# hongfz16/AvatarCLIP

Hardware: AMD Instinct MI355X
Metric: rays_per_sec_512x512_64spp_clip_guided_train_iter (higher is better)
Workload: dtype f16 (forward) / bf16 (gradient sweeps) MFMA operands, fp32 accumulate

## Files before the change

avatarclip_amd/csrc/avc_bwd_body.h:

```cpp
#pragma once
#include "avc_mlp.h"
constexpr int BWD_G = 4;
constexpr int BWD_WPB = 8;

template <typename P> __device__ __forceinline__ P launder(P p) {
  asm volatile("" : "+s"(p));
  return p;
}
template <typename V>
__device__ __forceinline__ V zero_frag() {
  V z;
#pragma unroll
  for (int j = 0; j < 8; ++j) z[j] = (typename MF<V>::S)0.f;
  return z;
}
__device__ __forceinline__ float second_term(float gbar_h, float g_a, float s) {
  const float r = s > 1e-30f ? __builtin_amdgcn_rcpf(s) : 0.f;
  return gbar_h * g_a * (AVC_BETA * (1.f - s) * r);
}
struct PF3 { h8 h0, h1; b8 b0, b1; h8 g0, g1; };

struct BwdArgs {
  PointSrc ps;
  long npts;
  const b8* Wb0;
  const float* T0;
  const float* d_sdf;
  const float* d_normal;
  const float* d_rgb;
  const float* rgb_fwd;
  const char* fpanels;
  char* gpanels;
  const unsigned short* masks;
  float* colsum;
};

#define AVC_CS_DUMMY 64
template <class N> struct ColSum {
  static constexpr int SLOT_FLOATS = PanelLayout<N>::CS_FLOATS + AVC_CS_DUMMY;
  static constexpr int LDS_BYTES = BWD_WPB * SLOT_FLOATS * 4;
};
typedef AVC_LDS float* cs_slot_t;
__device__ __forceinline__ float quad_xor1(float x) {
  return __builtin_bit_cast(float, __builtin_amdgcn_update_dpp(0, __builtin_bit_cast(int, x), 0xB1, 0xf, 0xf, true));
}
__device__ __forceinline__ float quad_xor2(float x) {
  return __builtin_bit_cast(float, __builtin_amdgcn_update_dpp(0, __builtin_bit_cast(int, x), 0x4E, 0xf, 0xf, true));
}
template <int NV>
__device__ __forceinline__ float transpose_sum(const float (&v)[NV], int lane) {
  static_assert(NV == 8 || NV == 16, "8 or 16 values per lane");
  float w[NV / 2];
  const bool b0 = lane & 1, b1 = lane & 2, b2 = lane & 4, b3 = lane & 8;
#pragma unroll
  for (int k = 0; k < NV / 2; ++k) w[k] = (b0 ? v[2 * k + 1] : v[2 * k]) + quad_xor1(b0 ? v[2 * k] : v[2 * k + 1]);
  float x[NV / 4];
#pragma unroll
  for (int k = 0; k < NV / 4; ++k) x[k] = (b1 ? w[2 * k + 1] : w[2 * k]) + quad_xor2(b1 ? w[2 * k] : w[2 * k + 1]);
  float y[NV / 8];
#pragma unroll
  for (int k = 0; k < NV / 8; ++k) y[k] = (b2 ? x[2 * k + 1] : x[2 * k]) + __shfl_xor(b2 ? x[2 * k] : x[2 * k + 1], 4);
  float z;
  if constexpr (NV == 16) z = (b3 ? y[1] : y[0]) + __shfl_xor(b3 ? y[0] : y[1], 8);
  else z = y[0] + __shfl_xor(y[0], 8);
  return z + __shfl_xor(z, 16);
}
template <class N, int NV>
__device__ __forceinline__ void col_sums(cs_slot_t slot, int lane, int base, const float (&v)[NV]) {
  const float total = transpose_sum<NV>(v, lane);
  const bool writer = (lane & 31) < NV;
  cs_slot_t dst = writer ? slot + base + (lane & (NV - 1)) : slot + PanelLayout<N>::CS_FLOATS + (lane & 63);
  *dst = *dst + total;
}
template <class N>
__device__ __forceinline__ cs_slot_t cs_init(char* lds_base, int wv, int lane) {
  cs_slot_t slot = (cs_slot_t)lds_base + wv * ColSum<N>::SLOT_FLOATS;
  for (int k = lane; k < ColSum<N>::SLOT_FLOATS; k += 64) slot[k] = 0.f;
  return slot;
}
template <class N>
__device__ __forceinline__ void cs_flush(cs_slot_t slot, float* out, long row, int lane) {
  asm volatile("s_waitcnt lgkmcnt(0)" ::: "memory");
  for (int k = lane; k < PanelLayout<N>::CS_FLOATS; k += 64) out[row * PanelLayout<N>::CS_FLOATS + k] = slot[k];
}

template <class N> struct BlkIn { b8 dof; unsigned m1[N::HT], m2[N::HT]; float dn[3], dsdf; };
template <class N>
__device__ __forceinline__ void load_blk_in(const BwdArgs& a, long blk, long nblk, int lane, BlkIn<N>& bi) {
  typedef PanelLayout<N> L;
  const int h = lane >> 5, p = lane & 31;
  long i = blk * 32 + p;
  const float vmask = i < a.npts ? 1.f : 0.f;
  if (i >= a.npts) i = a.npts - 1;
  bi.dof = zero_frag<b8>();
#pragma unroll
  for (int r = 0; r < 4; ++r) {
    const int ch = h ? 4 + r : r;
    const float c = (ch < 6) ? a.rgb_fwd[6 * i + (ch < 6 ? ch : 0)] : 0.f;
    const float dr = (ch < 6) ? a.d_rgb[6 * i + (ch < 6 ? ch : 0)] * vmask : 0.f;
    bi.dof[r] = (__bf16)(dr * c * (1.f - c));
  }
  const AVC_GLOBAL unsigned short* mk = as_global(a.masks) + (blk < nblk ? blk : nblk) * (long)L::MASK_U16 + lane;
#pragma unroll
  for (int t = 0; t < N::HT; ++t) {
    bi.m1[t] = mk[t * 64];
    bi.m2[t] = (N::NCMID == 1) ? mk[(N::HT + t) * 64] : 0u;
  }
#pragma unroll
  for (int c = 0; c < 3; ++c) bi.dn[c] = a.d_normal[3 * i + c] * vmask;
  bi.dsdf = a.d_sdf[i] * vmask;
}

struct NoRing {
  static constexpr bool on = false;
  template <class N> __device__ __forceinline__ void handoff(int, const b8 (&)[N::HK], long, int, int) const {}
};

template <class N, bool PIPE = false, class R>
__device__ __forceinline__ void bwd_sweeps(StageT<BWD_G>& sg, const BwdArgs& a, lds_tab_t Tl, long blk0, long nblk, int lane0,
                                           int wv, R& ring, cs_slot_t cs, BlkIn<N>* bip = nullptr, long blk0_next = 0) {
  typedef PanelLayout<N> L;
  constexpr AvcOffsets o = Off<N>::value;
  const PointSrc& ps = a.ps;
  const long npts = a.npts;
  const b8* Wb = launder(a.Wb0);
  lds_tab_t T = Tl;
  asm volatile("" : "+s"(T));
  int lane = lane0;
  asm volatile("" : "+v"(lane));
  const int h = lane >> 5, p = lane & 31;
  sg.lane = lane;
  const long blk = blk0 + wv;
  const long bsel = blk < nblk ? blk : nblk;
  const PanelPtr ftiles = panel_ptr(const_cast<char*>(a.fpanels) + bsel * (long)L::P_TILES * 2048, lane);
  const PanelPtr tiles = panel_ptr(a.gpanels + bsel * (long)L::G_TILES * 2048, lane);
  long i = blk * 32 + p;
  const bool valid = i < npts;
  if (!valid) i = npts - 1;
  const float vmask = valid ? 1.f : 0.f;
  float x[3];
  fetch_point(ps, i, x);
  float nbar[3];
  float dsdf_in;
  {
    BlkIn<N> bi_local;
    if constexpr (!PIPE) load_blk_in<N>(a, blk, nblk, lane, bi_local);
    BlkIn<N>& bi = PIPE ? *bip : bi_local;
    b8 dof[1];
    dof[0] = bi.dof;
    tile_store<false>(tiles, L::G_DO, dof[0], zero_frag<b8>());
    unsigned m1[N::HT], m2[N::HT];
#pragma unroll
    for (int t = 0; t < N::HT; ++t) { m1[t] = bi.m1[t]; m2[t] = bi.m2[t]; }
    const float dn_in[3] = {bi.dn[0], bi.dn[1], bi.dn[2]};
    dsdf_in = bi.dsdf;
#define AVC_RELU_BWD(OUT, MSK, PT)                                                                         \
  AVC_EPI(const unsigned bits = MSK[t];                                                                      \
          _Pragma("unroll") for (int j = 0; j < 8; ++j) {                                                    \
            OUT[2 * t][j] = (__bf16)(((bits >> relu_mask_bit(j)) & 1u) ? acc[j] : 0.f);                      \
            OUT[2 * t + 1][j] = (__bf16)(((bits >> relu_mask_bit(8 + j)) & 1u) ? acc[8 + j] : 0.f); }        \
          pin2(OUT[2 * t], OUT[2 * t + 1]);                                                                  \
          tile_store<false>(tiles, (PT) + t, OUT[2 * t], OUT[2 * t + 1]);)
    b8 dl[N::HK];
    b8 d1[N::HK];
    if constexpr (N::NCMID == 1) {
      layer_s1<b8, 1, N::HT>(sg, Wb, o.v[OFF_CHT], nxt<N, OFF_CM0T>(sg, Wb, o), dof, AVC_RELU_BWD(dl, m2, L::G_D2));
      layer_s1<b8, N::HK, N::HT>(sg, Wb, o.v[OFF_CM0T], nxt<N, OFF_C0T>(sg, Wb, o), dl, AVC_RELU_BWD(d1, m1, L::G_D1));
    } else {
      layer_s1<b8, 1, N::HT>(sg, Wb, o.v[OFF_CHT], nxt<N, OFF_C0T>(sg, Wb, o), dof, AVC_RELU_BWD(d1, m1, L::G_D1));
    }
    float dn_acc[3] = {0.f, 0.f, 0.f};
    layer_s1<b8, N::HK, N::HT + 1>(sg, Wb, o.v[OFF_C0T], nxt<N, OFF_W0G>(sg, Wb, o), d1, AVC_EPI(
      if (t < N::HT) {
        b8 f0, f1;
        _Pragma("unroll") for (int j = 0; j < 8; ++j) { f0[j] = (__bf16)acc[j]; f1[j] = (__bf16)acc[8 + j]; }
        pin2(f0, f1);
        tile_store<true>(tiles, L::G_DFEAT + (t < N::HT ? t : 0), f0, f1);
      } else {
        dn_acc[0] = acc[3]; dn_acc[1] = acc[0]; dn_acc[2] = acc[1];
      }
    ));
    {
      const float a3 = dn_acc[0], a0 = dn_acc[1], a1 = dn_acc[2];
      const float o3 = __shfl_xor(a3, 32), o0 = __shfl_xor(a0, 32), o1 = __shfl_xor(a1, 32);
      nbar[0] = valid ? dn_in[0] + (h ? o3 : a3) : 0.f;
      nbar[1] = valid ? dn_in[1] + (h ? a0 : o0) : 0.f;
      nbar[2] = valid ? dn_in[2] + (h ? a1 : o1) : 0.f;
    }
  }
  const float dsdf = dsdf_in;
  const float dsdfS = dsdf * AVC_S;
  {
    b8 fs = zero_frag<b8>();
    if (h == 0) {
      fs[0] = (__bf16)dsdf;
      fs[1] = (__bf16)(dsdf - (float)fs[0]);
    }
    tile_store<false>(tiles, L::G_SDF, fs, zero_frag<b8>());
  }
  b8 gbs[N::SK];
  b8 dfeat[N::HK];
  auto load_dfeat = [&]() __attribute__((always_inline)) {
#pragma unroll
    for (int t = 0; t < N::HT; ++t) {
      const FragPair<b8> d = tile_load<true, b8>(tiles, L::G_DFEAT + t);
      dfeat[2 * t] = d.a0;
      dfeat[2 * t + 1] = d.a1;
    }
  };
  {
    b8 gb0[3];
    {
      PE pe4;
      pe_compute(x, h, pe4);
      float g0[24];
#pragma unroll
      for (int q = 0; q < 24; ++q) {
        g0[q] = pe4.d[q] * nbar[q % 3];
        gb0[q >> 3][q & 7] = (__bf16)g0[q];
      }
#pragma unroll
      for (int s = 0; s < 3; ++s) {
        float v[8];
#pragma unroll
        for (int j = 0; j < 8; ++j) v[j] = g0[8 * s + j];
        col_sums<N, 8>(cs, lane, N::ST * 32 + (s * 2 + h) * 8, v);
      }
    }
    tile_store<false>(tiles, L::G_GB0, gb0[0], gb0[1]);
    tile_store<false>(tiles, L::G_GB0 + 1, gb0[2], zero_frag<b8>());
#define AVC_E_LOADH(PH) tile_load<false, h8>(ftiles, (PH) + t)
#define AVC_SECOND(OUT, PH, PT)                                                                              \
  AVC_PRE(return AVC_E_LOADH(PH);),                                                                          \
  AVC_EPID(FragPair<h8>, _Pragma("unroll") for (int j = 0; j < 8; ++j) {                                     \
            OUT[2 * t][j] = (__bf16)(acc[j] * sig_from_h((float)d.a0[j]));                                   \
            OUT[2 * t + 1][j] = (__bf16)(acc[8 + j] * sig_from_h((float)d.a1[j])); }                         \
          pin2(OUT[2 * t], OUT[2 * t + 1]);                                                                  \
          tile_store<true>(tiles, (PT) + t, OUT[2 * t], OUT[2 * t + 1]);)
#define AVC_SECOND_S(OUT, PH)                                                                                \
  AVC_PRE(return AVC_E_LOADH(PH);),                                                                          \
  AVC_EPID(FragPair<h8>, float v[16];                                                                        \
          _Pragma("unroll") for (int j = 0; j < 8; ++j) {                                                    \
            v[j] = acc[j] * sig_from_h((float)d.a0[j]);                                                      \
            v[8 + j] = acc[8 + j] * sig_from_h((float)d.a1[j]);                                              \
            OUT[2 * t][j] = (__bf16)v[j];                                                                    \
            OUT[2 * t + 1][j] = (__bf16)v[8 + j]; }                                                          \
          pin2(OUT[2 * t], OUT[2 * t + 1]);                                                                  \
          col_sums<N, 16>(cs, lane, (t * 2 + h) * 16, v);)
    b8 gb1[N::HK];
    layer_sq1<b8, 3, N::HT>(sg, Wb, o.v[OFF_W0G], nxt<N, OFF_WM0>(sg, Wb, o), gb0, AVC_SECOND(gb1, L::P_H1, L::G_GBH1));
    b8 gbm[N::HK];
    if constexpr (N::NMID == 2) {
      layer_sq1<b8, N::HK, N::HT>(sg, Wb, o.v[OFF_WM0], nxt<N, OFF_WM1>(sg, Wb, o), gb1, AVC_SECOND(gbm, L::P_HM, L::G_GBHM));
      b8 gbm1[N::HK];
      layer_sq1<b8, N::HK, N::HT>(sg, Wb, o.v[OFF_WM1], nxt<N, OFF_WS>(sg, Wb, o), gbm,
                                  AVC_SECOND(gbm1, L::P_HM + N::HT, L::G_GBHM + N::HT));
      layer_sq1<b8, N::HK, N::ST>(sg, Wb, o.v[OFF_WS], nxt<N, OFF_WLT>(sg, Wb, o), gbm1, AVC_SECOND_S(gbs, L::P_HS));
    } else {
      layer_sq1<b8, N::HK, N::HT>(sg, Wb, o.v[OFF_WM0], nxt<N, OFF_WS>(sg, Wb, o), gb1, AVC_SECOND(gbm, L::P_HM, L::G_GBHM));
      layer_sq1<b8, N::HK, N::ST>(sg, Wb, o.v[OFF_WS], nxt<N, OFF_WLT>(sg, Wb, o), gbm, AVC_SECOND_S(gbs, L::P_HS));
    }
  }
  {
    b8 as_[N::SK];
    load_dfeat();
#define AVC_F_LOADB(PB) tile_load<true, b8>(tiles, (PB) + t)
#define AVC_LOAD3(PH, PB, PG)                                                                               \
  AVC_PRE(PF3 d; { const FragPair<h8> a_ = tile_load<true, h8>(ftiles, (PH) + t); d.h0 = a_.a0; d.h1 = a_.a1; } \
          { const FragPair<b8> a_ = AVC_F_LOADB(PB); d.b0 = a_.a0; d.b1 = a_.a1; } \
          { const FragPair<h8> a_ = tile_load<true, h8>(ftiles, (PG) + t); d.g0 = a_.a0; d.g1 = a_.a1; } return d;)
#define AVC_LOAD3_S(PH, PG)                                                                                 \
  AVC_PRE(PF3 d; { const FragPair<h8> a_ = tile_load<true, h8>(ftiles, (PH) + t); d.h0 = a_.a0; d.h1 = a_.a1; } \
          d.b0 = gbs[2 * t]; d.b1 = gbs[2 * t + 1];                                                          \
          { const FragPair<h8> a_ = tile_load<true, h8>(ftiles, (PG) + t); d.g0 = a_.a0; d.g1 = a_.a1; } return d;)
    layer_sq1<b8, N::HK, N::ST>(sg, Wb, o.v[OFF_WLT], nxt<N, OFF_WST>(sg, Wb, o), dfeat,
      AVC_LOAD3_S(L::P_HS, L::P_GAS), AVC_EPID(PF3,
      float wa[16];
      load16(T + o.v[OFF_WL0_ACC], t, h, wa);
      _Pragma("unroll") for (int j = 0; j < 8; ++j) {
        const float s0 = sig_from_h((float)d.h0[j]), s1 = sig_from_h((float)d.h1[j]);
        as_[2 * t][j] = (__bf16)(second_term((float)d.b0[j], (float)d.g0[j], s0) + (acc[j] + wa[j] * dsdfS) * s0);
        as_[2 * t + 1][j] = (__bf16)(second_term((float)d.b1[j], (float)d.g1[j], s1) + (acc[8 + j] + wa[8 + j] * dsdfS) * s1);
      }
      pin2(as_[2 * t], as_[2 * t + 1]);
      tile_store<false>(tiles, L::G_ABS + t, as_[2 * t], as_[2 * t + 1]);
    ));
#define AVC_REVERSE(OUT, PH, PB, PG, PT, RINGED)                                                            \
  AVC_LOAD3(PH, PB, PG),                                                                                     \
  AVC_EPID(PF3, _Pragma("unroll") for (int j = 0; j < 8; ++j) {                                              \
            const float s0 = sig_from_h((float)d.h0[j]), s1 = sig_from_h((float)d.h1[j]);                    \
            OUT[2 * t][j] = (__bf16)(second_term((float)d.b0[j], (float)d.g0[j], s0) + acc[j] * s0);         \
            OUT[2 * t + 1][j] = (__bf16)(second_term((float)d.b1[j], (float)d.g1[j], s1) + acc[8 + j] * s1); } \
          pin2(OUT[2 * t], OUT[2 * t + 1]);                                                                  \
          if constexpr (!(RINGED)) tile_store<false>(tiles, (PT) + t, OUT[2 * t], OUT[2 * t + 1]);)
    b8 am[N::HK];
    b8 am0[N::HK];
    const Next first = nxt<N, OFF_CHT>(sg, a.Wb0, o);
#define AVC_F_LASTHOOK AVC_HOOK(if constexpr (PIPE) load_blk_in<N>(a, blk0_next + wv, nblk, lane, *bip);)
    if constexpr (N::NMID == 2) {
      layer_sq1<b8, N::SK, N::HT>(sg, Wb, o.v[OFF_WST], nxt<N, OFF_WM1T>(sg, Wb, o), as_,
                                 AVC_REVERSE(am, L::P_HM + N::HT, L::G_GBHM + N::HT, L::P_GAM + N::HT, L::G_ABM + N::HT, R::on));
      if constexpr (R::on) ring.template handoff<N>(1, am, blk0, lane, wv);
      layer_sq1<b8, N::HK, N::HT>(sg, Wb, o.v[OFF_WM1T], nxt<N, OFF_WM0T>(sg, Wb, o), am,
                                 AVC_REVERSE(am0, L::P_HM, L::G_GBHM, L::P_GAM, L::G_ABM, R::on));
      if constexpr (R::on) ring.template handoff<N>(0, am0, blk0, lane, wv);
      layer_sq1<b8, N::HK, N::HT>(sg, Wb, o.v[OFF_WM0T], first, am0, AVC_REVERSE(am, L::P_H1, L::G_GBH1, L::P_GA1, L::G_AB1, false), AVC_F_LASTHOOK);
    } else {
      layer_sq1<b8, N::SK, N::HT>(sg, Wb, o.v[OFF_WST], nxt<N, OFF_WM0T>(sg, Wb, o), as_,
                                 AVC_REVERSE(am, L::P_HM, L::G_GBHM, L::P_GAM, L::G_ABM, R::on));
      if constexpr (R::on) ring.template handoff<N>(0, am, blk0, lane, wv);
      layer_sq1<b8, N::HK, N::HT>(sg, Wb, o.v[OFF_WM0T], first, am, AVC_REVERSE(am0, L::P_H1, L::G_GBH1, L::P_GA1, L::G_AB1, false), AVC_F_LASTHOOK);
    }
  }
#undef AVC_RELU_BWD
#undef AVC_SECOND
#undef AVC_LOAD3
#undef AVC_LOAD3_S
#undef AVC_F_LOADB
#undef AVC_E_LOADH
#undef AVC_SECOND_S
#undef AVC_F_LASTHOOK
#undef AVC_REVERSE
}
```

avatarclip_amd/csrc/avc_mlp_bwd.hip:

```cpp
#include "avc_bwd_body.h"
#include "../../include/avc.h"

template <class N>
__global__ __launch_bounds__(64 * BWD_WPB) void mlp_bwd_kernel(BwdArgs a) {
  extern __shared__ __attribute__((aligned(16))) char lds[];
  typedef StageT<BWD_G> ST;
  constexpr AvcOffsets o = Off<N>::value;
  static_assert(BWD_WPB >= 4 && BWD_WPB % 4 == 0, "stage_issue's turns need a multiple of 4 wavefronts per workgroup");
  const int lane0 = threadIdx.x & 63;
  const int wv = threadIdx.x >> 6;
  const long nblk = (a.npts + 31) >> 5;
  ST sg = stage_init<BWD_G>(lds);
  stage_issue(sg, nxt<N, OFF_CHT>(sg, a.Wb0, o), 0);
  const lds_tab_t Tl = tab_to_lds(lds + ST::LDS_BYTES, a.T0, o.v[OFF_TAB_END]);
  const cs_slot_t cs = cs_init<N>(lds + ST::LDS_BYTES + AVC_TAB_LDS_BYTES, wv, lane0);
  __syncthreads();
  NoRing ring;
  BlkIn<N> bi;
  load_blk_in<N>(a, (long)blockIdx.x * BWD_WPB + wv, nblk, lane0, bi);
  for (long blk0 = (long)blockIdx.x * BWD_WPB; blk0 < nblk; blk0 += (long)gridDim.x * BWD_WPB)
    bwd_sweeps<N, true>(sg, a, Tl, blk0, nblk, lane0, wv, ring, cs, &bi, blk0 + (long)gridDim.x * BWD_WPB);
  cs_flush<N>(cs, a.colsum, (long)blockIdx.x * BWD_WPB + wv, lane0);
}

extern "C" int avc_bwd_colsum_floats(int net) { return net == AVC_NET_FULL ? PanelLayout<NetFull>::CS_FLOATS : PanelLayout<NetSmall>::CS_FLOATS; }
extern "C" long avc_bwd_colsum_rows(long npts, long max_waves) {
  const long nblk = (npts + 31) / 32;
  long ngroups = (nblk + BWD_WPB - 1) / BWD_WPB, maxg = max_waves / BWD_WPB;
  if (maxg < 1) maxg = 1;
  long grid = ngroups < maxg ? ngroups : maxg;
  if (grid < 1) grid = 1;
  return grid * BWD_WPB;
}

extern "C" int avc_render_points_bwd(int net, const float* pts, const float* rays_o, const float* rays_d, const float* z,
                                     int S, int ldz, float sample_dist, long npts, const void* wbf16, const float* tab,
                                     const int* offs, const float* d_sdf, const float* d_normal, const float* d_rgb,
                                     const float* rgb_fwd, const void* fpanels, void* gpanels, const void* masks, float* colsum,
                                     long max_waves, void* stream) {
  if (npts <= 0) return 0;
  if (!fpanels || !gpanels || !masks || !rgb_fwd || !colsum) { avc_set_error("avc_render_points_bwd: fpanels / gpanels / masks / rgb_fwd / colsum == NULL"); return 1; }
  if (!(net == AVC_NET_FULL ? offsets_match<NetFull>(offs) : offsets_match<NetSmall>(offs))) {
    avc_set_error("packed-blob offsets differ from the compiled-in table (regenerate csrc/avc_offsets_gen.h)");
    return 1;
  }
  PointSrc ps{pts, rays_o, rays_d, z, S, ldz, pts ? 0 : 1, sample_dist};
  const long nblk = (npts + 31) / 32;
  long ngroups = (nblk + BWD_WPB - 1) / BWD_WPB;
  long maxg = max_waves / BWD_WPB;
  if (maxg < 1) maxg = 1;
  int grid = (int)(ngroups < maxg ? ngroups : maxg);
  if (grid < 1) grid = 1;
  hipStream_t s = (hipStream_t)stream;
  const int lds_bytes = StageT<BWD_G>::LDS_BYTES + AVC_TAB_LDS_BYTES + ColSum<NetFull>::LDS_BYTES;
  if (offs[OFF_TAB_END] * 4 > AVC_TAB_LDS_BYTES) { avc_set_error("fp32 table does not fit its LDS window"); return 1; }
  static unsigned long long attr_seen = 0;
  if (avc_first_use_on_device(attr_seen)) {
    (void)hipFuncSetAttribute((const void*)mlp_bwd_kernel<NetFull>, hipFuncAttributeMaxDynamicSharedMemorySize, lds_bytes);
    (void)hipFuncSetAttribute((const void*)mlp_bwd_kernel<NetSmall>, hipFuncAttributeMaxDynamicSharedMemorySize, lds_bytes);
  }
  const BwdArgs args{ps, npts, (const b8*)wbf16, tab, d_sdf, d_normal, d_rgb, rgb_fwd, (const char*)fpanels, (char*)gpanels,
                     (const unsigned short*)masks, colsum};
  if (net == AVC_NET_FULL)
    hipLaunchKernelGGL((mlp_bwd_kernel<NetFull>), dim3(grid), dim3(64 * BWD_WPB), lds_bytes, s, args);
  else if (net == AVC_NET_SMALL)
    hipLaunchKernelGGL((mlp_bwd_kernel<NetSmall>), dim3(grid), dim3(64 * BWD_WPB), lds_bytes, s, args);
  else { avc_set_error("unknown net id"); return 1; }
  return avc_check_launch("avc_render_points_bwd");
}
```

avatarclip_amd/csrc/avc_wgrad.hip:

```cpp
#include "avc_common.h"
#include "../../include/avc.h"

#include "avc_wgrad_body.h"

template <int NI, int NK>
__device__ __forceinline__ void weight_grad_body(char* lds, const WgRegions& rg, int pa, int ta_n, int pb,
                                                 int tb_n, int type_a, int type_b, long nblk, float* __restrict__ partial,
                                                 float* __restrict__ bias_partial, int out_elems, int bias_elems, int WA) {
  const int lane = threadIdx.x & 63;
  const int wv = __builtin_amdgcn_readfirstlane((int)(threadIdx.x >> 6));
  const int WB = 8 / WA;
  const int wa = wv % WA, wb = wv / WA;
  const int split = blockIdx.x, nsplit = gridDim.x;
  const long b0 = nblk * split / nsplit, b1 = nblk * (split + 1) / nsplit;
  const int ntile = ta_n + tb_n;
  const int nchunk = ntile * 2;
  const int my_chunks = (nchunk - wv + 7) >> 3;
  constexpr int slot_bytes = WG_BUF_BYTES, depth = WG_DEPTH;
  const int src_lo = ((lane >> 2) & 3) * 32 + 4 * (lane >> 4) + (lane & 3);
  const char* const base_a = (type_a ? rg.base[1] : rg.base[0]) + (long)pa * 2048;
  const char* const base_b = (type_b ? rg.base[1] : rg.base[0]) + (long)pb * 2048;
  const long stride_a = type_a ? rg.stride[1] : rg.stride[0], stride_b = type_b ? rg.stride[1] : rg.stride[0];
  auto issue = [&](long blk, int slot) {
    for (int c = wv; c < nchunk; c += 8) {
      const int tix = c >> 1;
      const char* tb_ = tix < ta_n ? base_a + blk * stride_a + (long)tix * 2048 : base_b + blk * stride_b + (long)(tix - ta_n) * 2048;
      const char* g = tb_ + (src_lo + (c & 1) * 16) * 16;
      __builtin_amdgcn_global_load_lds((const __attribute__((address_space(1))) void*)g,
                                       (__attribute__((address_space(3))) void*)(lds + slot * slot_bytes + c * 1024), 16, 0, WG_DMA_AUX);
    }
  };
  const int lane_off = (((lane >> 5) * 2) * 16 + (((lane >> 4) & 1) * 2 + (lane & 1)) * 4 + ((lane & 15) >> 2)) * 16 + 8 * ((lane & 3) >> 1);
  facc acc[NI * NK];
#pragma unroll
  for (int q = 0; q < NI * NK; ++q)
#pragma unroll
    for (int r = 0; r < 16; ++r) acc[q][r] = 0.f;
  float bsum[NI];
#pragma unroll
  for (int i = 0; i < NI; ++i) bsum[i] = 0.f;
  for (int d = 0; d < depth - 1; ++d)
    if (b0 + d < b1) issue(b0 + d, d);
  int slot = 0;
  for (long blk = b0; blk < b1; ++blk) {
    long younger = b1 - 1 - blk;
    if (younger > depth - 2) younger = depth - 2;
    wait_vmcnt((int)younger * my_chunks);
    asm volatile("s_waitcnt lgkmcnt(0)" ::: "memory");
    __builtin_amdgcn_s_barrier();
    __builtin_amdgcn_sched_barrier(0);
    if (blk + depth - 1 < b1) { int ns = slot + depth - 1; if (ns >= depth) ns -= depth; issue(blk + depth - 1, ns); }
    lds_char* buf = (lds_char*)(lds + slot * slot_bytes) + lane_off;
    b8 a[NI][2];
#pragma unroll
    for (int i = 0; i < NI; ++i) {
      const int ta = wa + WA * i;
      if (ta < ta_n) {
        a[i][0] = tr_frag(buf + ta * 2048, 0);
        a[i][1] = tr_frag(buf + ta * 2048, 1);
      }
    }
    b8 bv[NK][2];
#pragma unroll
    for (int k = 0; k < NK; ++k) {
      const int tb = wb + WB * k;
      if (tb < tb_n) {
        bv[k][0] = tr_frag(buf + (ta_n + tb) * 2048, 0);
        bv[k][1] = tr_frag(buf + (ta_n + tb) * 2048, 1);
      }
    }
    if (type_a == 0) {
#pragma unroll
      for (int i = 0; i < NI; ++i) { a[i][0] = f16_to_bf16(a[i][0]); a[i][1] = f16_to_bf16(a[i][1]); }
    }
    if (type_b == 0) {
#pragma unroll
      for (int k = 0; k < NK; ++k) { bv[k][0] = f16_to_bf16(bv[k][0]); bv[k][1] = f16_to_bf16(bv[k][1]); }
    }
#pragma unroll
    for (int i = 0; i < NI; ++i) {
      if (wa + WA * i < ta_n) {
        if (bias_partial && wb == i) {
#pragma unroll
          for (int j = 0; j < 8; ++j) bsum[i] += (float)a[i][0][j] + (float)a[i][1][j];
        }
#pragma unroll
        for (int k = 0; k < NK; ++k) {
          if (wb + WB * k < tb_n) {
            acc[i * NK + k] = MF<b8>::mma(a[i][0], bv[k][0], acc[i * NK + k]);
            acc[i * NK + k] = MF<b8>::mma(a[i][1], bv[k][1], acc[i * NK + k]);
          }
        }
      }
    }
    if (++slot == depth) slot = 0;
  }
  float* dst = partial + (long)split * out_elems;
#pragma unroll
  for (int i = 0; i < NI; ++i) {
    const int ta = wa + WA * i;
    if (ta >= ta_n) continue;
#pragma unroll
    for (int k = 0; k < NK; ++k) {
      const int tb = wb + WB * k;
      if (tb >= tb_n) continue;
      f4* d4 = reinterpret_cast<f4*>(dst + ((long)(ta * tb_n + tb) * 64 + lane) * 16);
#pragma unroll
      for (int q = 0; q < 4; ++q) {
        f4 v;
        v[0] = acc[i * NK + k][4 * q]; v[1] = acc[i * NK + k][4 * q + 1]; v[2] = acc[i * NK + k][4 * q + 2]; v[3] = acc[i * NK + k][4 * q + 3];
        d4[q] = v;
      }
    }
    if (bias_partial && wb == i) {
      const float s = xhalf_sum(bsum[i]);
      if (lane < 32) bias_partial[(long)split * bias_elems + ta * 32 + lane] = s;
    }
  }
}

__device__ __forceinline__ void weight_grad_body_9x9(char* lds, const WgRegions& rg, int pa, int pb, int type_a,
                                                     int type_b, long nblk, float* __restrict__ partial,
                                                     float* __restrict__ bias_partial, int out_elems, int bias_elems) {
  constexpr int TA = 9, TB = 9, NT = TA + TB;
  const int lane = threadIdx.x & 63;
  const int wv = __builtin_amdgcn_readfirstlane((int)(threadIdx.x >> 6));
  const int wa = wv & 3, wb = wv >> 2;
  const int split = blockIdx.x, nsplit = gridDim.x;
  const long b0 = nblk * split / nsplit, b1 = nblk * (split + 1) / nsplit;
  constexpr int nchunk = NT * 2;
  const int my_chunks = (nchunk - wv + 7) >> 3;
  const int src_lo = ((lane >> 2) & 3) * 32 + 4 * (lane >> 4) + (lane & 3);
  const char* const base_a = (type_a ? rg.base[1] : rg.base[0]) + (long)pa * 2048;
  const char* const base_b = (type_b ? rg.base[1] : rg.base[0]) + (long)pb * 2048;
  const long stride_a = type_a ? rg.stride[1] : rg.stride[0], stride_b = type_b ? rg.stride[1] : rg.stride[0];
  auto issue = [&](long blk, int slot) {
    for (int c = wv; c < nchunk; c += 8) {
      const int tix = c >> 1;
      const char* tb_ = tix < TA ? base_a + blk * stride_a + (long)tix * 2048 : base_b + blk * stride_b + (long)(tix - TA) * 2048;
      const char* g = tb_ + (src_lo + (c & 1) * 16) * 16;
      __builtin_amdgcn_global_load_lds((const __attribute__((address_space(1))) void*)g,
                                       (__attribute__((address_space(3))) void*)(lds + slot * WG_BUF_BYTES + c * 1024), 16, 0, WG_DMA_AUX);
    }
  };
  const int lane_off = (((lane >> 5) * 2) * 16 + (((lane >> 4) & 1) * 2 + (lane & 1)) * 4 + ((lane & 15) >> 2)) * 16 + 8 * ((lane & 3) >> 1);
  facc acc[10], ex[2];
#pragma unroll
  for (int q = 0; q < 10; ++q)
#pragma unroll
    for (int r = 0; r < 16; ++r) acc[q][r] = 0.f;
#pragma unroll
  for (int q = 0; q < 2; ++q)
#pragma unroll
    for (int r = 0; r < 16; ++r) ex[q][r] = 0.f;
  float bsum[2] = {0.f, 0.f}, xsum = 0.f;
  const bool has_x = wb == 1 || wa == 0;
  const int xk = wb == 1 ? wa : 4;
  for (int d = 0; d < WG_DEPTH - 1; ++d)
    if (b0 + d < b1) issue(b0 + d, d);
  int slot = 0;
  for (long blk = b0; blk < b1; ++blk) {
    long younger = b1 - 1 - blk;
    if (younger > WG_DEPTH - 2) younger = WG_DEPTH - 2;
    wait_vmcnt((int)younger * my_chunks);
    asm volatile("s_waitcnt lgkmcnt(0)" ::: "memory");
    __builtin_amdgcn_s_barrier();
    __builtin_amdgcn_sched_barrier(0);
    if (blk + WG_DEPTH - 1 < b1) issue(blk + WG_DEPTH - 1, (slot + WG_DEPTH - 1) % WG_DEPTH);
    lds_char* buf = (lds_char*)(lds + slot * WG_BUF_BYTES) + lane_off;
    auto load_b = [&](int tb, b8& f0, b8& f1) {
      f0 = tr_frag(buf + (TA + tb) * 2048, 0);
      f1 = tr_frag(buf + (TA + tb) * 2048, 1);
    };
    b8 a[2][2], sa[2], c0, c1, n0, n1;
    load_b(wb, c0, c1);
    n0 = c0; n1 = c1;
#pragma unroll
    for (int i = 0; i < 2; ++i) {
      a[i][0] = tr_frag(buf + (wa + 4 * i) * 2048, 0);
      a[i][1] = tr_frag(buf + (wa + 4 * i) * 2048, 1);
    }
    if (has_x) { sa[0] = tr_frag(buf + 8 * 2048, 0); sa[1] = tr_frag(buf + 8 * 2048, 1); }
    if (type_a == 0) {
#pragma unroll
      for (int i = 0; i < 2; ++i) { a[i][0] = f16_to_bf16(a[i][0]); a[i][1] = f16_to_bf16(a[i][1]); }
      if (has_x) { sa[0] = f16_to_bf16(sa[0]); sa[1] = f16_to_bf16(sa[1]); }
    }
    if (bias_partial) {
#pragma unroll
      for (int i = 0; i < 2; ++i)
        if (wb == i) {
#pragma unroll
          for (int j = 0; j < 8; ++j) bsum[i] += (float)a[i][0][j] + (float)a[i][1][j];
        }
    }
    if (bias_partial && wv == 4) {
#pragma unroll
      for (int j = 0; j < 8; ++j) xsum += (float)sa[0][j] + (float)sa[1][j];
    }
#pragma unroll
    for (int k = 0; k < 6; ++k) {
      const int tb_next = (k + 1 < 5) ? wb + 2 * (k + 1) : 2 * wa;
      const bool next_ok = (k + 1 < 5) ? (tb_next < TB) : (k + 1 == 5 && wb == 1);
      if (next_ok) load_b(tb_next, n0, n1);
      asm volatile("" : "+v"(n0), "+v"(n1));
      const bool cur_ok = (k < 5) ? (wb + 2 * k < TB) : (wb == 1);
      if (cur_ok) {
        if (type_b == 0) { c0 = f16_to_bf16(c0); c1 = f16_to_bf16(c1); }
        if (k < 5) {
          acc[k] = MF<b8>::mma(a[0][0], c0, acc[k]);
          acc[k] = MF<b8>::mma(a[0][1], c1, acc[k]);
          acc[5 + k] = MF<b8>::mma(a[1][0], c0, acc[5 + k]);
          acc[5 + k] = MF<b8>::mma(a[1][1], c1, acc[5 + k]);
          if (has_x && k == xk) {
            ex[0] = MF<b8>::mma(sa[0], c0, ex[0]);
            ex[0] = MF<b8>::mma(sa[1], c1, ex[0]);
          }
        } else {
          ex[1] = MF<b8>::mma(sa[0], c0, ex[1]);
          ex[1] = MF<b8>::mma(sa[1], c1, ex[1]);
        }
      }
      c0 = n0; c1 = n1;
    }
    slot = (slot + 1) % WG_DEPTH;
  }
  float* dst = partial + (long)split * out_elems;
  auto store_tile = [&](int ta, int tb, const facc& v16) {
    f4* d4 = reinterpret_cast<f4*>(dst + ((long)(ta * TB + tb) * 64 + lane) * 16);
#pragma unroll
    for (int q = 0; q < 4; ++q) {
      f4 v;
      v[0] = v16[4 * q]; v[1] = v16[4 * q + 1]; v[2] = v16[4 * q + 2]; v[3] = v16[4 * q + 3];
      d4[q] = v;
    }
  };
#pragma unroll
  for (int k = 0; k < 5; ++k) {
    if (wb + 2 * k < TB) {
      store_tile(wa, wb + 2 * k, acc[k]);
      store_tile(wa + 4, wb + 2 * k, acc[5 + k]);
    }
  }
  if (has_x) store_tile(8, wb + 2 * xk, ex[0]);
  if (wb == 1) store_tile(8, 2 * wa, ex[1]);
  if (bias_partial) {
#pragma unroll
    for (int i = 0; i < 2; ++i) {
      if (wb == i) {
        const float sx = xhalf_sum(bsum[i]);
        if (lane < 32) bias_partial[(long)split * bias_elems + (wa + 4 * i) * 32 + lane] = sx;
      }
    }
    if (wv == 4) {
      const float sx = xhalf_sum(xsum);
      if (lane < 32) bias_partial[(long)split * bias_elems + 8 * 32 + lane] = sx;
    }
  }
}

#define WG_MAX_PAIRS 24
struct WgPairs { int v[WG_MAX_PAIRS][8]; };
__global__ __launch_bounds__(512) void weight_grad_all_kernel(WgRegions rg, WgPairs pp, long nblk,
                                                              float* __restrict__ partial, float* __restrict__ bias_partial,
                                                              int out_elems, int bias_elems) {
  extern __shared__ __attribute__((aligned(16))) char lds[];
  const int* d = pp.v[blockIdx.y];
  float* bp = d[5] >= 0 ? bias_partial + d[5] : nullptr;
#define WG_ARGS lds, rg, d[0], d[1], d[2], d[3], d[6], d[7], nblk, partial + d[4], bp, out_elems, bias_elems
  if (d[1] > 1 && d[3] > 2 && d[3] <= 8) {
    if (d[7] == 0) weight_grad_body<4, 2>(WG_ARGS, 2);
    else weight_grad_body<2, 4>(WG_ARGS, 4);
  } else if (d[1] == 9 && d[3] == 9) {
    weight_grad_body_9x9(lds, rg, d[0], d[2], d[6], d[7], nblk, partial + d[4], bp, out_elems, bias_elems);
  } else if (d[1] > 1 && d[3] > 8) {
    weight_grad_body<2, 5>(WG_ARGS, 4);
  } else if (d[1] > 1) {
    weight_grad_body<1, 2>(WG_ARGS, 8);
  } else {
    weight_grad_body<1, 2>(WG_ARGS, 1);
  }
#undef WG_ARGS
}

extern "C" int avc_weight_grad_all(const void* fpanels, int ftiles, const void* gpanels, int gtiles, int npairs, const int* pairs,
                                   long nblk, float* partial, float* bias_partial, int nsplit, int out_stride, int bias_stride,
                                   void* stream) {
  if (nblk <= 0 || npairs <= 0) return 0;
  if (!fpanels || !gpanels) { avc_set_error("avc_weight_grad_all: fpanels / gpanels == NULL"); return 1; }
  if (npairs > WG_MAX_PAIRS) { avc_set_error("avc_weight_grad_all: too many pairs"); return 1; }
  WgPairs pp;
  for (int i = 0; i < npairs; ++i) {
    for (int k = 0; k < 8; ++k) pp.v[i][k] = pairs[i * 8 + k];
    const bool merged = pp.v[i][1] == 9 && pp.v[i][3] == 9;
    if (!merged && (pp.v[i][1] < 1 || pp.v[i][1] > 8 || pp.v[i][3] < 1 || pp.v[i][3] > WG_TB_MAX)) {
      avc_set_error("avc_weight_grad_all: 1 <= ta <= 8, 1 <= tb <= 9 (or the 9 x 9 product)");
      return 1;
    }
  }
  if (nsplit < 1) nsplit = 1;
  const int lds_bytes = WG_DEPTH * WG_BUF_BYTES;
  static unsigned long long attr_seen = 0;
  if (avc_first_use_on_device(attr_seen)) {
    (void)hipFuncSetAttribute((const void*)weight_grad_all_kernel, hipFuncAttributeMaxDynamicSharedMemorySize, lds_bytes);
  }
  WgRegions rg;
  rg.base[0] = (const char*)fpanels; rg.stride[0] = (long)ftiles * 2048;
  rg.base[1] = (const char*)gpanels; rg.stride[1] = (long)gtiles * 2048;
  hipLaunchKernelGGL(weight_grad_all_kernel, dim3(nsplit, npairs), dim3(512), lds_bytes, (hipStream_t)stream, rg, pp, nblk, partial,
                     bias_partial, out_stride, bias_stride);
  return avc_check_launch("avc_weight_grad_all");
}

__global__ __launch_bounds__(256) void wgrad_reduce_kernel(const float* __restrict__ partial, const float* __restrict__ bpartial, int ns,
                                                           long stride, long bstride, int gout4, int gbias4, float* __restrict__ acc,
                                                           int accumulate) {
  const int j = blockIdx.x * 256 + threadIdx.x;
  if (j >= gout4 + gbias4) return;
  const f4* src = j < gout4 ? reinterpret_cast<const f4*>(partial) + j : reinterpret_cast<const f4*>(bpartial) + (j - gout4);
  const long st4 = (j < gout4 ? stride : bstride) >> 2;
  f4 a = {0.f, 0.f, 0.f, 0.f};
  int s = 0;
  for (; s + 8 <= ns; s += 8) {
    f4 v[8];
#pragma unroll
    for (int u = 0; u < 8; ++u) v[u] = __builtin_nontemporal_load(src + (long)(s + u) * st4);
#pragma unroll
    for (int u = 0; u < 8; ++u) a += v[u];
  }
  for (; s < ns; ++s) a += __builtin_nontemporal_load(src + (long)s * st4);
  f4* out = reinterpret_cast<f4*>(acc) + j;
  if (accumulate) a += *out;
  *out = a;
}
__global__ __launch_bounds__(256) void wgrad_unpack_kernel(const float* __restrict__ acc, const int* __restrict__ off, const int* __restrict__ src,
                                                           const float* __restrict__ scale, int nparam, float* __restrict__ grad) {
  const int t = blockIdx.x * 256 + threadIdx.x;
  if (t >= nparam) return;
  float g = 0.f;
  for (int k = off[t]; k < off[t + 1]; ++k) g += acc[src[k]] * scale[k];
  grad[t] = g;
}
extern "C" int avc_weight_grad_reduce(const float* partial, const float* bias_partial, int nsplit, int out_stride, int bias_stride,
                                      int gout_size, int gbias_size, float* acc, int accumulate, void* stream) {
  if ((gout_size & 3) || (gbias_size & 3) || (out_stride & 3) || (bias_stride & 3)) {
    avc_set_error("avc_weight_grad_reduce: sizes and strides must be multiples of 4 floats");
    return 1;
  }
  if (nsplit < 1 || !partial || !acc || (gbias_size && !bias_partial)) { avc_set_error("avc_weight_grad_reduce: bad arguments"); return 1; }
  const int n4 = (gout_size + gbias_size) / 4;
  hipLaunchKernelGGL(wgrad_reduce_kernel, dim3((n4 + 255) / 256), dim3(256), 0, (hipStream_t)stream, partial, bias_partial, nsplit,
                     (long)out_stride, (long)bias_stride, gout_size / 4, gbias_size / 4, acc, accumulate);
  return avc_check_launch("avc_weight_grad_reduce");
}
extern "C" int avc_weight_grad_unpack(const float* acc, const int* off, const int* src, const float* scale, int nparam, float* grad,
                                      void* stream) {
  if (nparam <= 0) return 0;
  if (!acc || !off || !src || !scale || !grad) { avc_set_error("avc_weight_grad_unpack: NULL buffer"); return 1; }
  hipLaunchKernelGGL(wgrad_unpack_kernel, dim3((nparam + 255) / 256), dim3(256), 0, (hipStream_t)stream, acc, off, src, scale, nparam, grad);
  return avc_check_launch("avc_weight_grad_unpack");
}
```

avatarclip_amd/engine.py:

```python
import ctypes
import os
import weakref

import numpy as np
import torch

from . import lib as L
from . import packing as PK


class _DevLayout:

    _cache = {}

    def __init__(self, lay: PK.Layout, device):
        t = lambda a, dt=None: torch.from_numpy(np.ascontiguousarray(a)).to(device)
        self.lay = lay
        self.idx16 = t(lay.idx16)
        self.scale16 = t(lay.scale16)
        self.idx32 = t(lay.idx32)
        self.scale32 = t(lay.scale32)
        self.un_src = t(lay.un_src)
        self.un_tgt = t(lay.un_tgt)
        self.un_scale = t(lay.un_scale)
        self.ub_src = t(lay.ub_src)
        self.ub_tgt = t(lay.ub_tgt)
        tgt = np.concatenate([lay.un_tgt, lay.ub_tgt]).astype(np.int64)
        src = np.concatenate([lay.un_src, np.asarray(lay.ub_src, np.int64) + lay.gout_size]).astype(np.int64)
        scl = np.concatenate([lay.un_scale, np.ones(len(lay.ub_tgt), np.float32)]).astype(np.float32)
        order = np.argsort(tgt, kind="stable")
        off = np.zeros(lay.nparam + 1, np.int64)
        np.cumsum(np.bincount(tgt, minlength=lay.nparam), out=off[1:])
        self.csr_off, self.csr_src, self.csr_scale = t(off.astype(np.int32)), t(src[order].astype(np.int32)), t(scl[order])
        self.cs_src, self.cs_tgt, self.cs_scale = t(lay.cs_src), t(lay.cs_tgt), t(lay.cs_scale)
        self._offsets_arr = (ctypes.c_int * PK.OFF_COUNT)(*[int(v) for v in lay.offsets])
        self.offsets = ctypes.cast(self._offsets_arr, ctypes.c_void_p)

    @classmethod
    def get(cls, spec, device):
        key = (spec.H, spec.NMID, spec.NCMID, str(device))
        if key not in cls._cache:
            cls._cache[key] = cls(PK.layout_for(spec), device)
        return cls._cache[key]


FUSED_PACK = os.environ.get("AVC_FUSED_PACK", "1") != "0"


class Packed:

    def __init__(self, dl: _DevLayout, flatP: torch.Tensor):
        self.dl = dl
        if flatP.is_cuda and FUSED_PACK:
            f = flatP.detach().float().contiguous()
            n16, n32 = dl.idx16.numel(), dl.idx32.numel()
            self.w_f16 = torch.empty(n16, dtype=torch.float16, device=f.device)
            self.w_bf16 = torch.empty(n16, dtype=torch.bfloat16, device=f.device)
            self.tab = torch.empty(n32, dtype=torch.float32, device=f.device)
            L.check(L.load().avc_pack_params(L.ptr(f), f.numel(), L.ptr(dl.idx16), L.ptr(dl.scale16), n16, L.ptr(dl.idx32), L.ptr(dl.scale32), n32,
                                             L.ptr(self.w_f16), L.ptr(self.w_bf16), L.ptr(self.tab), L.stream()), "avc_pack_params")
            return
        pz = torch.cat([flatP.detach().float(), flatP.new_zeros(1)])
        w = pz[dl.idx16] * dl.scale16
        self.w_f16 = w.to(torch.float16).contiguous()
        self.w_bf16 = w.to(torch.bfloat16).contiguous()
        self.tab = (pz[dl.idx32] * dl.scale32).contiguous()


def flatten_dense_torch(sdf_net, col_net, spec: PK.NetSpec) -> torch.Tensor:
    parts = []
    for W, b in sdf_net.dense():
        parts += [W.reshape(-1), b.reshape(-1)]
    if col_net is not None:
        for W, b in col_net.dense():
            parts += [W.reshape(-1), b.reshape(-1)]
    else:
        lay = PK.layout_for(spec)
        n_sdf = sum(int(np.prod(s)) for n, s in lay.shapes if n.startswith("sdf."))
        parts.append(parts[0].new_zeros(lay.nparam - n_sdf))
    return torch.cat(parts)


def _dense_layers(sdf_net, col_net, lay):
    out = []
    n_sdf = sdf_net.num_layers - 1
    for l in range(n_sdf):
        out.append((getattr(sdf_net, "lin%d" % l), lay.pbase["sdf.W%d" % l], lay.pbase["sdf.b%d" % l]))
    if col_net is not None:
        nh = col_net.num_layers - 2
        for l in range(nh):
            out.append((getattr(col_net, "lin%d" % l), lay.pbase["col.W%d" % l], lay.pbase["col.b%d" % l]))
        last = getattr(col_net, "lin%d" % nh)
        H = last.weight_v.shape[1] if hasattr(last, "weight_v") else last.weight.shape[1]
        out.append((last, lay.pbase["col.Wh"], lay.pbase["col.bh"]))
        if col_net.extra_color:
            out.append((col_net.extra_lin, lay.pbase["col.Wh"] + 3 * H, lay.pbase["col.bh"] + 3))
    return out


class DenseParamsFn(torch.autograd.Function):

    @staticmethod
    def forward(ctx, meta, *tensors):
        lay, offs = meta
        n = len(offs)
        dev = tensors[0].device
        flat = torch.zeros(lay.nparam, device=dev, dtype=torch.float32)
        vs, gs, bs = tensors[0::3], tensors[1::3], tensors[2::3]
        PA = ctypes.c_void_p * n
        arr = lambda ts: PA(*[(t.data_ptr() if t.numel() else None) for t in ts])
        ctx.rows = (ctypes.c_int * n)(*[v.shape[0] for v in vs])
        ctx.cols = (ctypes.c_int * n)(*[v.shape[1] for v in vs])
        ctx.w_off = (ctypes.c_long * n)(*[o[0] for o in offs])
        ctx.b_off = (ctypes.c_long * n)(*[o[1] for o in offs])
        ctx.n = n
        lib = L.load()
        assert all(t.is_contiguous() and t.dtype == torch.float32 for t in tensors)
        L.check(lib.avc_dense_params_fwd(n, arr(vs), arr(gs), arr(bs), ctx.rows, ctx.cols, ctx.w_off, ctx.b_off, L.ptr(flat), L.stream()),
                "avc_dense_params_fwd")
        ctx.save_for_backward(*tensors)
        return flat

    @staticmethod
    def backward(ctx, dflat):
        tensors = ctx.saved_tensors
        n = ctx.n
        vs, gs, bs = tensors[0::3], tensors[1::3], tensors[2::3]
        dflat = dflat.contiguous().float()
        outs = [torch.empty_like(t) for t in tensors]
        PA = ctypes.c_void_p * n
        arr = lambda ts: PA(*[(t.data_ptr() if t.numel() else None) for t in ts])
        L.check(L.load().avc_dense_params_bwd(n, arr(vs), arr(gs), arr(outs[0::3]), arr(outs[1::3]), arr(outs[2::3]), ctx.rows, ctx.cols,
                                              ctx.w_off, ctx.b_off, L.ptr(dflat), L.stream()), "avc_dense_params_bwd")
        return (None,) + tuple(o if t.numel() else None for o, t in zip(outs, tensors))


def flatten_dense(sdf_net, col_net, spec: PK.NetSpec) -> torch.Tensor:
    p0 = next(sdf_net.parameters())
    if p0.device.type != "cuda":
        return flatten_dense_torch(sdf_net, col_net, spec)
    lay = PK.layout_for(spec)
    tensors, offs = [], []
    empty = p0.new_zeros(0)
    for lin, w_off, b_off in _dense_layers(sdf_net, col_net, lay):
        if hasattr(lin, "weight_g"):
            tensors += [lin.weight_v, lin.weight_g, lin.bias if lin.bias is not None else empty]
        else:
            tensors += [lin.weight, empty, lin.bias if lin.bias is not None else empty]
        offs.append((int(w_off), int(b_off)))
    return DenseParamsFn.apply((lay, offs), *tensors)


def plan_panels(R, S, budget, blk_f, blk_g, slab_blocks, min_slab_blocks):
    nb = lambda rays: (rays * S + 31) // 32 + 1
    rays_of = lambda blocks: min(R, max(32, blocks * 32 // S // 32 * 32))
    blocks = slab_blocks
    slab = rays_of(blocks)
    while nb(R) * blk_f + nb(slab) * blk_g > budget and blocks > min_slab_blocks:
        blocks //= 2
        slab = rays_of(blocks)
    if nb(R) * blk_f + nb(slab) * blk_g <= budget:
        return R, slab
    if nb(slab) * (blk_f + blk_g) > budget:
        slab = max(32, (budget // (blk_f + blk_g) - 1) * 32 // S // 32 * 32)
    chunk = max(slab, ((budget - nb(slab) * blk_g) // blk_f - 1) * 32 // S // 32 * 32)
    return min(chunk, R), min(slab, R)


class Engine:
    _by_net = weakref.WeakKeyDictionary()
    PROFILE = False
    prof_events = []
    WG_BLOCKS_PER_SPLIT = int(os.environ.get("AVC_WG_BLOCKS_PER_SPLIT", "256"))
    WG_MAX_SPLITS = int(os.environ.get("AVC_WG_MAX_SPLITS", "256"))
    FUSED_WG_TAIL = os.environ.get("AVC_FUSED_WG_TAIL", "1") != "0"
    MAX_FWD_WAVES = 2048
    MAX_BWD_WAVES = 2048
    SDF_BIAS_FP32 = os.environ.get("AVC_SDF_BIAS_FP32", "1") != "0"
    RING = os.environ.get("AVC_BWD_RING", "0") != "0"
    RING_CPT = int(os.environ.get("AVC_RING_CPT", "2"))
    RING_SLOTS = int(os.environ.get("AVC_RING_SLOTS", "6"))
    RING_CHECK = os.environ.get("AVC_RING_CHECK", "0") != "0"
    PANEL_BYTES_BUDGET = int(os.environ.get("AVC_PANEL_GIB", "224")) << 30
    SLAB_BLOCKS = int(os.environ.get("AVC_SLAB_BLOCKS", str(512 * 1024)))
    MIN_SLAB_BLOCKS = 32 * 1024

    def __init__(self, spec: PK.NetSpec, device):
        if device.type != "cuda":
            raise RuntimeError("avatarclip_amd runs its hot path on an MI355X; got device %s (no CPU fallback)" % device)
        self.spec = spec
        self.device = device
        self.lib = L.load()
        self.dl = _DevLayout.get(spec, device)
        self.net = spec.net_id
        assert self.lib.avc_num_offsets() == PK.OFF_COUNT
        self.fwd_tiles = self.lib.avc_fwd_panel_tiles(self.net)
        self.grad_tiles = self.lib.avc_grad_panel_tiles(self.net)
        assert (self.fwd_tiles, self.grad_tiles) == (self.dl.lay.panel["FTILES"], self.dl.lay.panel["GTILES"]), \
            "panel layout mismatch between packing.py and csrc/avc_mlp.h"
        assert self.lib.avc_bwd_colsum_floats(self.net) == self.dl.lay.cs_size, "column-sum layout mismatch between packing.py and csrc/avc_mlp.h"
        self._colsum = None
        self.mask_u16 = self.lib.avc_mask_u16_per_block(self.net)
        self.fwd_scr_bytes = self.lib.avc_fwd_scratch_bytes_per_wave(self.net)
        self._fwd_scratch = None
        self._fpanels = None
        self._gpanels = None
        self._partials = None
        self._bpartials = None
        self._masks = None
        self._pairs_host = PK.region_local_pairs(self.dl.lay)
        self._sdf_bias0 = int(self.dl.lay.pbase["sdf.b%d" % (spec.NMID + 2)])
        self._packed_key = None
        self._packed = None
        self._panel_owner = None
        self._ring = None
        self.ring_stats = None

    @classmethod
    def for_networks(cls, sdf_net, col_net):
        eng = cls._by_net.get(sdf_net)
        if eng is None:
            col_conf = col_net.conf if col_net is not None else dict(
                d_hidden=sdf_net.conf["d_hidden"], n_layers=2 if sdf_net.conf["d_hidden"] == 256 else 1,
                mode="no_view_dir", multires_view=0)
            spec = PK.spec_from_conf(sdf_net.conf, col_conf)
            eng = cls(spec, next(sdf_net.parameters()).device)
            cls._by_net[sdf_net] = eng
        return eng

    class _Timed:
        def __init__(self, name, npts):
            self.name, self.npts = name, npts

        def __enter__(self):
            if Engine.PROFILE:
                self.e0 = torch.cuda.Event(enable_timing=True)
                self.e1 = torch.cuda.Event(enable_timing=True)
                self.e0.record()
            return self

        def __exit__(self, *a):
            if Engine.PROFILE:
                self.e1.record()
                Engine.prof_events.append((self.name, self.npts, self.e0, self.e1))
            return False

    def pack(self, flatP: torch.Tensor) -> Packed:
        last = getattr(self, "_last_pack", None)
        if last is not None and last[0]() is flatP and last[1] == flatP._version:
            return last[2]
        pk = Packed(self.dl, flatP)
        self._last_pack = (weakref.ref(flatP), flatP._version, pk)
        return pk

    def colsum_scratch(self):
        if getattr(self, "_colsum_scratch", None) is None:
            self._colsum_scratch = torch.zeros(self.lib.avc_colsum_scratch_bytes(), dtype=torch.uint8, device=self.device)
        return self._colsum_scratch

    def _grow(self, attr, nbytes, dtype=torch.uint8):
        buf = getattr(self, attr)
        esz = torch.empty(0, dtype=dtype).element_size()
        n = nbytes // esz
        if buf is None or buf.numel() < n:
            n = ((n * esz + (1 << 21) - 1) >> 21 << 21) // esz
            buf = None
            setattr(self, attr, None)
            torch.cuda.empty_cache()
            buf = torch.zeros(n, dtype=dtype, device=self.device)
            setattr(self, attr, buf)
        return buf

    def _bufs_f(self, nblk_chunk):
        return (self._grow("_fpanels", (nblk_chunk + 1) * self.fwd_tiles * 2048),
                self._grow("_masks", (nblk_chunk + 1) * self.mask_u16 * 2, torch.int16))

    def _bufs_g(self, nblk_slab):
        return self._grow("_gpanels", (nblk_slab + 1) * self.grad_tiles * 2048)

    def _ring_setup(self):
        if not L.has_ring():
            raise RuntimeError("AVC_BWD_RING=1 needs libavc_ring.so (python -m avatarclip_amd.build --ring; AVC_LIB_NAME=libavc_ring.so): the "
                               "role-specialised backward is an experiment that is not part of libavc.so (include/avc_ring.h)")
        key = (self.RING_CPT, self.RING_SLOTS)
        if self._ring is not None and self._ring["key"] == key:
            return self._ring
        lay, lib = self.dl.lay, self.lib
        ht = self.spec.H // 32
        ntypes = lib.avc_bwd_ring_types(self.net)
        assert ntypes == self.spec.NMID
        ring_rows, pb, offs = [], [], []
        for m in range(ntypes):
            row = [i for i, pr in enumerate(lay.pairs) if pr[0] == lay.panel["ABM"] + m * ht and pr[6] == 1]
            assert len(row) == 1
            pr = lay.pairs[row[0]]
            assert pr[1] == ht and pr[3] == ht and pr[7] == 0 and pr[5] >= 0, "ring products are HT x HT with an F-region B operand and a bias"
            ring_rows.append(row[0]); pb.append(int(pr[2])); offs.append((int(pr[4]), int(pr[5])))
        rest = np.ascontiguousarray(np.delete(self._pairs_host, ring_rows, axis=0))
        nrow = 8 * self.RING_CPT
        dev = self.device
        self._ring = dict(
            key=key, ntypes=ntypes, ht=ht, offs=offs, rest=rest,
            ctl=torch.zeros(lib.avc_bwd_ring_ctl_bytes() // 4, dtype=torch.int32, device=dev),
            payload=torch.empty(lib.avc_bwd_ring_payload_bytes(self.net, ntypes, self.RING_SLOTS), dtype=torch.uint8, device=dev),
            partial=torch.zeros(ntypes, nrow, ht * ht * 1024, dtype=torch.float32, device=dev),
            bias=torch.zeros(ntypes, nrow, ht * 32, dtype=torch.float32, device=dev),
            pb=(ctypes.c_int * ntypes)(*pb),
            err=torch.zeros((), dtype=torch.int32, device=dev),
            grid=torch.cuda.get_device_properties(dev).multi_processor_count)
        return self._ring

    def _held_bytes(self):
        return sum(b.numel() * b.element_size() for b in (self._fpanels, self._gpanels, self._masks) if b is not None)

    def plan(self, R, S):
        key = (R, S, self.PANEL_BYTES_BUDGET, self.SLAB_BLOCKS)
        if getattr(self, "_plan_key", None) == key:
            chunk, slab = self._plan_val
            if chunk < R or (self._fpanels is not None and self._fpanels.numel() >= ((R * S + 31) // 32 + 1) * self.fwd_tiles * 2048):
                return self._plan_val
        nb_all = (R * S + 31) // 32 + 1
        if (self._fpanels is not None and self._gpanels is not None and nb_all <= self.SLAB_BLOCKS
                and self._fpanels.numel() >= nb_all * self.fwd_tiles * 2048 and self._gpanels.numel() >= nb_all * self.grad_tiles * 2048
                and self._held_bytes() <= self.PANEL_BYTES_BUDGET):
            return R, R
        budget = max(min(self.PANEL_BYTES_BUDGET, (torch.cuda.mem_get_info(self.device)[0] + self._held_bytes()) * 8 // 10), 1 << 26)
        self._plan_key = key
        self._plan_val = plan_panels(R, S, budget, self.fwd_tiles * 2048 + self.mask_u16 * 2, self.grad_tiles * 2048,
                                     self.SLAB_BLOCKS, self.MIN_SLAB_BLOCKS)
        return self._plan_val

    def rays_per_chunk(self, R, S):
        return self.plan(R, S)[0]

    def sdf_rays(self, pk: Packed, rays_o, rays_d, z, sdf_out=None, slot=None, ld_out=0):
        R, S = z.shape
        if sdf_out is None:
            sdf_out = torch.empty(R, S, device=self.device, dtype=torch.float32)
        with Engine._Timed("avc_sdf_forward", R * S):
            L.check(self.lib.avc_sdf_forward(self.net, None, L.ptr(rays_o), L.ptr(rays_d), L.ptr(z), S, z.stride(0), R * S,
                                             L.ptr(pk.w_f16), L.ptr(pk.tab), self.dl.offsets, L.ptr(sdf_out),
                                             L.ptr(slot), ld_out, L.stream()), "avc_sdf_forward")
        return sdf_out

    def sdf_pts(self, pk: Packed, pts):
        pts = pts.contiguous().float()
        out = torch.empty(pts.shape[0], 1, device=self.device, dtype=torch.float32)
        L.check(self.lib.avc_sdf_forward(self.net, L.ptr(pts), None, None, None, 1, 1, pts.shape[0], L.ptr(pk.w_f16),
                                         L.ptr(pk.tab), self.dl.offsets, L.ptr(out), None, 0, L.stream()),
                "avc_sdf_forward")
        return out

    def upsample_step(self, rays_o, rays_d, z, sdf, m, inv_s):
        R, n = z.shape
        z_out = torch.empty(R, n + m, device=self.device, dtype=torch.float32)
        sdf_out = torch.empty(R, n + m, device=self.device, dtype=torch.float32)
        z_new = torch.empty(R, m, device=self.device, dtype=torch.float32)
        slot = torch.empty(R, m, device=self.device, dtype=torch.int32)
        lanes = 64 if os.environ.get("AVC_UPSAMPLE_GROUP", "1") == "0" else 0
        L.check(self.lib.avc_upsample_step_lanes(L.ptr(rays_o), L.ptr(rays_d), L.ptr(z), L.ptr(sdf), R, n, m, float(inv_s),
                                                 L.ptr(z_out), L.ptr(sdf_out), L.ptr(z_new), L.ptr(slot), lanes, L.stream()),
                "avc_upsample_step")
        return z_out, sdf_out, z_new, slot

    def points_fwd(self, pk: Packed, rays_o, rays_d, z, sample_dist):
        R, S = z.shape
        N = R * S
        sdf = torch.empty(R, S, device=self.device, dtype=torch.float32)
        nrm = torch.empty(R, S, 3, device=self.device, dtype=torch.float32)
        rgb = torch.empty(R, S, 6, device=self.device, dtype=torch.float32)
        if self._fwd_scratch is None:
            self._fwd_scratch = torch.empty(self.MAX_FWD_WAVES * self.fwd_scr_bytes, dtype=torch.uint8, device=self.device)
        with Engine._Timed("avc_render_points_fwd", N):
            L.check(self.lib.avc_render_points_fwd(self.net, None, L.ptr(rays_o), L.ptr(rays_d), L.ptr(z), S, z.stride(0),
                                                   float(sample_dist), N, L.ptr(pk.w_f16), L.ptr(pk.tab), self.dl.offsets,
                                                   L.ptr(sdf), L.ptr(nrm), L.ptr(rgb), self.MAX_FWD_WAVES, L.ptr(self._fwd_scratch),
                                                   L.stream()), "avc_render_points_fwd")
        return sdf, nrm, rgb

    def points_fwd_train(self, pk: Packed, rays_o, rays_d, z, sample_dist, r0=0, r1=None, out=None):
        R, S = z.shape
        r1 = R if r1 is None else r1
        if out is None:
            out = (torch.empty(R, S, device=self.device, dtype=torch.float32), torch.empty(R, S, 3, device=self.device, dtype=torch.float32),
                   torch.empty(R, S, 6, device=self.device, dtype=torch.float32))
        sdf, nrm, rgb = out
        npts = (r1 - r0) * S
        panels, masks = self._bufs_f((npts + 31) // 32)
        esz = 4
        with Engine._Timed("avc_render_points_fwd_train", npts):
            L.check(self.lib.avc_render_points_fwd_train(
                self.net, None, rays_o.data_ptr() + r0 * 3 * esz, rays_d.data_ptr() + r0 * 3 * esz,
                z.data_ptr() + r0 * z.stride(0) * esz, S, z.stride(0), float(sample_dist), npts, L.ptr(pk.w_f16), L.ptr(pk.tab),
                self.dl.offsets, sdf.data_ptr() + r0 * S * esz, nrm.data_ptr() + r0 * S * 3 * esz, rgb.data_ptr() + r0 * S * 6 * esz,
                self.MAX_FWD_WAVES, L.ptr(panels), L.ptr(masks), L.stream()), "avc_render_points_fwd_train")
        return out

    def composite_fwd(self, sdf, nrm, rgb, z, rays_o, rays_d, inv_s, sample_dist, cos_anneal, bg, bg_mode):
        R, S = z.shape
        dev, f32 = self.device, torch.float32
        color = torch.empty(R, 3, device=dev, dtype=f32)
        extra = torch.empty(R, 3, device=dev, dtype=f32)
        weights = torch.empty(R, S, device=dev, dtype=f32)
        cdf = torch.empty(R, S, device=dev, dtype=f32)
        mid_z = torch.empty(R, S, device=dev, dtype=f32)
        inside = torch.empty(R, S, device=dev, dtype=f32)
        eik = torch.empty(R, 2, device=dev, dtype=f32)
        wstat = torch.empty(2, R, device=dev, dtype=f32)
        nsum = torch.empty(R, 3, device=dev, dtype=f32)
        L.check(self.lib.avc_composite_fwd(L.ptr(sdf), L.ptr(nrm), L.ptr(rgb), L.ptr(z), L.ptr(rays_o), L.ptr(rays_d), R, S,
                                           L.ptr(inv_s), float(sample_dist), float(cos_anneal), L.ptr(bg), bg_mode,
                                           L.ptr(color), L.ptr(extra), L.ptr(weights), L.ptr(cdf), L.ptr(mid_z),
                                           L.ptr(inside), L.ptr(eik), L.ptr(wstat), L.ptr(nsum), L.stream()), "avc_composite_fwd")
        return color, extra, weights, cdf, mid_z, inside, eik, wstat, nsum

    def composite_bwd(self, sdf, nrm, rgb, z, rays_o, rays_d, inv_s, sample_dist, cos_anneal, bg, bg_mode, d_color,
                      d_extra, d_w, d_n_up, eik_scale, d_wsum=None, d_nsum=None):
        R, S = z.shape
        dev, f32 = self.device, torch.float32
        d_sdf = torch.empty(R, S, device=dev, dtype=f32)
        d_n = torch.empty(R, S, 3, device=dev, dtype=f32)
        d_rgb = torch.empty(R, S, 6, device=dev, dtype=f32)
        d_inv = torch.empty(R, device=dev, dtype=f32)
        L.check(self.lib.avc_composite_bwd(L.ptr(sdf), L.ptr(nrm), L.ptr(rgb), L.ptr(z), L.ptr(rays_o), L.ptr(rays_d), R, S,
                                           L.ptr(inv_s), float(sample_dist), float(cos_anneal), L.ptr(bg), bg_mode,
                                           L.ptr(d_color), L.ptr(d_extra), L.ptr(d_w), L.ptr(d_n_up), L.ptr(d_wsum), L.ptr(d_nsum),
                                           L.ptr(eik_scale), L.ptr(d_sdf), L.ptr(d_n), L.ptr(d_rgb), L.ptr(d_inv), L.stream()),
                "avc_composite_bwd")
        return d_sdf, d_n, d_rgb, d_inv

    def points_bwd(self, pk: Packed, rays_o, rays_d, z, sample_dist, d_sdf, d_n, d_rgb, rgb, panels_valid=False):
        lay = self.dl.lay
        R, S = z.shape
        rays_per_chunk, rays_per_slab = self.plan(R, S)
        if rays_per_chunk < R:
            panels_valid = False
        rg = self._ring_setup() if self.RING else None
        fused_tail = rg is None and self.FUSED_WG_TAIL and lay.gout_size % 4 == 0 and lay.gbias_size % 4 == 0
        if fused_tail:
            gacc = torch.empty(lay.gout_size + lay.gbias_size, device=self.device, dtype=torch.float32)
            nslab = 0
        else:
            gout = torch.zeros(lay.gout_size, device=self.device, dtype=torch.float32)
            gbias = torch.zeros(max(lay.gbias_size, 1), device=self.device, dtype=torch.float32)
        if self._partials is None:
            self._partials = torch.empty(256, lay.gout_size, device=self.device, dtype=torch.float32)
            self._bpartials = torch.empty(256, max(lay.gbias_size, 1), device=self.device, dtype=torch.float32)
        st = L.stream()
        esz = 4
        scratch_out = None
        if rg is not None:
            rg["err"].zero_()
        pairs_host = rg["rest"] if rg is not None else self._pairs_host
        cs_rows = int(self.lib.avc_bwd_colsum_rows(min(R, rays_per_slab) * S, self.MAX_BWD_WAVES)) if rg is None else 8 * rg["grid"]
        if self._colsum is None or self._colsum.shape[0] < cs_rows:
            self._colsum = torch.zeros(cs_rows, lay.cs_size, device=self.device, dtype=torch.float32)
        cs_total = None
        for c0 in range(0, R, rays_per_chunk):
            c1 = min(R, c0 + rays_per_chunk)
            if not panels_valid:
                if scratch_out is None:
                    scratch_out = (torch.empty(R, S, device=self.device), torch.empty(R, S, 3, device=self.device),
                                   torch.empty(R, S, 6, device=self.device))
                self.points_fwd_train(pk, rays_o, rays_d, z, sample_dist, c0, c1, out=scratch_out)
            fpanels, masks = self._bufs_f(((c1 - c0) * S + 31) // 32)
            for s0 in range(c0, c1, rays_per_slab):
                s1 = min(c1, s0 + rays_per_slab)
                npts = (s1 - s0) * S
                nblk = (npts + 31) // 32
                assert ((s0 - c0) * S) % 32 == 0, "slabs start on a 32-point block of their chunk"
                fblk0 = (s0 - c0) * S // 32
                fptr = fpanels.data_ptr() + fblk0 * self.fwd_tiles * 2048
                mptr = masks.data_ptr() + fblk0 * self.mask_u16 * 2
                gpanels = self._bufs_g(nblk)
                bwd_args = (self.net, None, rays_o.data_ptr() + s0 * 3 * esz, rays_d.data_ptr() + s0 * 3 * esz,
                            z.data_ptr() + s0 * z.stride(0) * esz, S, z.stride(0), float(sample_dist), npts, L.ptr(pk.w_bf16), L.ptr(pk.tab),
                            self.dl.offsets, d_sdf.data_ptr() + s0 * S * esz, d_n.data_ptr() + s0 * S * 3 * esz,
                            d_rgb.data_ptr() + s0 * S * 6 * esz, rgb.data_ptr() + s0 * S * 6 * esz, fptr, L.ptr(gpanels), mptr, L.ptr(self._colsum))
                if rg is None:
                    rows = int(self.lib.avc_bwd_colsum_rows(npts, self.MAX_BWD_WAVES))
                    with Engine._Timed("avc_render_points_bwd", npts):
                        L.check(self.lib.avc_render_points_bwd(*bwd_args, self.MAX_BWD_WAVES, st), "avc_render_points_bwd")
                else:
                    rows = 8 * rg["grid"]
                    self._colsum[:rows].zero_()
                    rg["partial"].zero_()
                    rg["bias"].zero_()
                    with Engine._Timed("avc_render_points_bwd_ring", npts):
                        L.check(self.lib.avc_render_points_bwd_ring(
                            *bwd_args, L.ptr(rg["ctl"]), L.ptr(rg["payload"]), L.ptr(rg["partial"]), L.ptr(rg["bias"]), rg["pb"],
                            rg["ntypes"], self.RING_CPT, self.RING_SLOTS, rg["grid"], st), "avc_render_points_bwd_ring")
                    rg["err"] += rg["ctl"][64]
                    if self.RING_CHECK:
                        torch.cuda.synchronize()
                        self.ring_stats = rg["ctl"][96:112].cpu().numpy().view(np.uint64).copy()
                        if int(rg["ctl"][64]) != 0:
                            raise RuntimeError("avc_render_points_bwd_ring: %d spin time-out(s), first site %d, counters %s"
                                               % (int(rg["ctl"][64]), int(rg["ctl"][65]), self.ring_stats))
                cs_slab = self._colsum[:rows].sum(0)
                cs_total = cs_slab if cs_total is None else cs_total + cs_slab
                ns = max(1, min(self.WG_MAX_SPLITS, nblk // self.WG_BLOCKS_PER_SPLIT, nblk))
                with Engine._Timed("avc_weight_grad(all pairs)", npts):
                    L.check(self.lib.avc_weight_grad_all(fptr, self.fwd_tiles, L.ptr(gpanels), self.grad_tiles, len(pairs_host),
                                                         pairs_host.ctypes.data, nblk, L.ptr(self._partials),
                                                         L.ptr(self._bpartials), ns, self._partials.stride(0),
                                                         self._bpartials.stride(0), st), "avc_weight_grad_all")
                    if fused_tail:
                        L.check(self.lib.avc_weight_grad_reduce(L.ptr(self._partials), L.ptr(self._bpartials), ns, self._partials.stride(0),
                                                                self._bpartials.stride(0), lay.gout_size, lay.gbias_size, L.ptr(gacc),
                                                                int(nslab > 0), st), "avc_weight_grad_reduce")
                        nslab += 1
                        continue
                    po, pb_ = self._partials[:ns].sum(0), self._bpartials[:ns].sum(0)
                    if rg is not None:
                        for m, (o_off, b_off) in enumerate(rg["offs"]):
                            po[o_off:o_off + rg["partial"].shape[2]] = rg["partial"][m].sum(0)
                            pb_[b_off:b_off + rg["bias"].shape[2]] = rg["bias"][m].sum(0)
                    gout += po
                    gbias += pb_
        self._panel_owner = None
        if fused_tail:
            grad = torch.empty(lay.nparam, device=self.device, dtype=torch.float32)
            if nslab == 0:
                grad.zero_()
            else:
                L.check(self.lib.avc_weight_grad_unpack(L.ptr(gacc), L.ptr(self.dl.csr_off), L.ptr(self.dl.csr_src), L.ptr(self.dl.csr_scale),
                                                        lay.nparam, L.ptr(grad), st), "avc_weight_grad_unpack")
        else:
            grad = torch.zeros(lay.nparam, device=self.device, dtype=torch.float32)
            grad.index_add_(0, self.dl.un_tgt, gout[self.dl.un_src] * self.dl.un_scale)
            if lay.gbias_size:
                grad.index_add_(0, self.dl.ub_tgt, gbias[self.dl.ub_src])
        if cs_total is not None:
            grad.index_add_(0, self.dl.cs_tgt, cs_total[self.dl.cs_src] * self.dl.cs_scale)
        if self.SDF_BIAS_FP32:
            grad[self._sdf_bias0] = d_sdf.sum()
        if rg is not None:
            grad = torch.where(rg["err"] != 0, torch.full_like(grad, float("nan")), grad)
        return grad


class RenderCoreFn(torch.autograd.Function):

    @staticmethod
    def forward(ctx, flatP, inv_s, eng, rays_o, rays_d, z_vals, sample_dist, cos_anneal, bg, bg_mode):
        pk = eng.pack(flatP)
        inv_s_d = inv_s.detach().float().contiguous()
        R, S = z_vals.shape
        needs_grad = bool(ctx.needs_input_grad[0] or ctx.needs_input_grad[1])
        ctx.panel_token = None
        if needs_grad and eng.plan(R, S)[0] >= R:
            sdf, nrm, rgb = eng.points_fwd_train(pk, rays_o, rays_d, z_vals, sample_dist)
            ctx.panel_token = eng._panel_owner = object()
        else:
            sdf, nrm, rgb = eng.points_fwd(pk, rays_o, rays_d, z_vals, sample_dist)
        color, extra, weights, cdf, mid_z, inside, eik, wstat, nsum = eng.composite_fwd(
            sdf, nrm, rgb, z_vals, rays_o, rays_d, inv_s_d, sample_dist, cos_anneal, bg, bg_mode)
        wsum, wmax = wstat[0].reshape(R, 1), wstat[1].reshape(R, 1)
        eo = torch.empty(2, device=eik.device, dtype=torch.float32)
        L.check(eng.lib.avc_colsum(L.ptr(eik), R, 2, 1, L.ptr(eo), L.ptr(eng.colsum_scratch()), L.stream()), "avc_colsum")
        gerr, eik_den = eo[0], eo[1]
        ctx.eng, ctx.pk = eng, pk
        ctx.consts = (sample_dist, cos_anneal, bg_mode)
        ctx.save_for_backward(rays_o, rays_d, z_vals, sdf, nrm, rgb, inv_s_d, eik_den, bg if bg is not None else inv_s_d)
        ctx.has_bg = bg is not None
        ctx.mark_non_differentiable(cdf, mid_z, inside, sdf, wmax)
        ctx.set_materialize_grads(False)
        return color, extra, weights, nrm, gerr, cdf, mid_z, inside, sdf, wsum, wmax, nsum

    @staticmethod
    def backward(ctx, d_color, d_extra, d_weights, d_nrm, d_gerr, d_cdf=None, d_midz=None, d_inside=None, d_sdf_out=None,
                 d_wsum=None, d_wmax=None, d_nsum=None):
        eng, pk = ctx.eng, ctx.pk
        rays_o, rays_d, z_vals, sdf, nrm, rgb, inv_s_d, eik_den, bg = ctx.saved_tensors
        if not ctx.has_bg:
            bg = None
        sample_dist, cos_anneal, bg_mode = ctx.consts
        R, S = z_vals.shape
        zeros = lambda *s: torch.zeros(*s, device=z_vals.device, dtype=torch.float32)
        d_color = d_color.contiguous().float() if d_color is not None else zeros(R, 3)
        d_extra = d_extra.contiguous().float() if d_extra is not None else zeros(R, 3)
        d_weights = d_weights.contiguous().float() if d_weights is not None else None
        d_nrm = d_nrm.contiguous().float() if d_nrm is not None else None
        d_wsum = d_wsum.contiguous().float().reshape(R) if d_wsum is not None else None
        d_nsum = d_nsum.contiguous().float() if d_nsum is not None else None
        d_gerr = d_gerr if d_gerr is not None else zeros(())
        eik_scale = (d_gerr.float() / eik_den).reshape(1).contiguous()
        d_sdf, d_n, d_rgb, d_inv = eng.composite_bwd(sdf, nrm, rgb, z_vals, rays_o, rays_d, inv_s_d, sample_dist,
                                                     cos_anneal, bg, bg_mode, d_color, d_extra, d_weights, d_nrm, eik_scale,
                                                     d_wsum, d_nsum)
        valid = ctx.panel_token is not None and eng._panel_owner is ctx.panel_token
        grad = eng.points_bwd(pk, rays_o, rays_d, z_vals, sample_dist, d_sdf, d_n, d_rgb, rgb, panels_valid=valid)
        d_inv_s = torch.empty(1, device=d_inv.device, dtype=torch.float32)
        L.check(eng.lib.avc_colsum(L.ptr(d_inv), R, 1, 0, L.ptr(d_inv_s), L.ptr(eng.colsum_scratch()), L.stream()), "avc_colsum")
        return grad, d_inv_s, None, None, None, None, None, None, None, None
```

avatarclip_amd/lib.py:

```python
import ctypes
import os

import torch

from . import build as _build

_lib = None
ABI_VERSION = 3

c_int, c_long, c_float, c_double, c_void_p = ctypes.c_int, ctypes.c_long, ctypes.c_float, ctypes.c_double, ctypes.c_void_p
P = c_void_p

_SIGS = {
    "avc_version": (c_int, []),
    "avc_num_offsets": (c_int, []),
    "avc_sdf_forward": (c_int, [c_int, P, P, P, P, c_int, c_int, c_long, P, P, P, P, P, c_int, P]),
    "avc_upsample_step": (c_int, [P, P, P, P, c_int, c_int, c_int, c_float, P, P, P, P, P]),
    "avc_upsample_step_lanes": (c_int, [P, P, P, P, c_int, c_int, c_int, c_float, P, P, P, P, c_int, P]),
    "avc_render_points_fwd": (c_int, [c_int, P, P, P, P, c_int, c_int, c_float, c_long, P, P, P, P, P, P, c_long, P, P]),
    "avc_fwd_scratch_bytes_per_wave": (c_long, [c_int]),
    "avc_composite_fwd": (c_int, [P, P, P, P, P, P, c_int, c_int, P, c_float, c_float, P, c_int, P, P, P, P, P, P, P, P, P, P]),
    "avc_composite_bwd": (c_int, [P, P, P, P, P, P, c_int, c_int, P, c_float, c_float, P, c_int, P, P, P, P, P, P, P,
                                  P, P, P, P, P]),
    "avc_render_points_fwd_train": (c_int, [c_int, P, P, P, P, c_int, c_int, c_float, c_long, P, P, P, P, P, P, c_long, P, P, P]),
    "avc_fwd_panel_tiles": (c_int, [c_int]),
    "avc_grad_panel_tiles": (c_int, [c_int]),
    "avc_mask_u16_per_block": (c_int, [c_int]),
    "avc_render_points_bwd": (c_int, [c_int, P, P, P, P, c_int, c_int, c_float, c_long, P, P, P, P, P, P, P, P, P, P, P, c_long, P]),
    "avc_bwd_colsum_floats": (c_int, [c_int]),
    "avc_bwd_colsum_rows": (c_long, [c_long, c_long]),
    "avc_mc_classify": (c_int, [P, c_int, c_int, c_int, c_float, P, P, P, P]),
    "avc_mc_emit": (c_int, [P, c_int, c_int, c_int, c_float, P, P, P, P, P, P, P, P, P]),
    "avc_text_attention_fwd": (c_int, [P, P, c_int, c_int, c_int, c_int, c_int, P]),
    "avc_vit_linear": (c_int, [P, P, P, P, P, P, c_int, c_int, c_int, c_int, P, P]),
    "avc_vit_linear_bwd_gelu": (c_int, [P, P, P, P, c_int, c_int, c_int, P, P]),
    "avc_vit_workspace_bytes": (c_long, [c_int, c_int]),
    "avc_vit_ln_pack": (c_int, [P, P, P, c_float, c_int, c_int, P, P]),
    "avc_vit_linear_packed": (c_int, [P, P, P, P, P, P, c_int, c_int, c_int, c_int, P]),
    "avc_vit_pack": (c_int, [P, P, P, c_int, c_int, P]),
    "avc_vit_attention_bwd_packed": (c_int, [P, P, P, c_int, c_int, c_int, c_int, P]),
    "avc_vit_linear_small": (c_int, [P, P, P, P, P, P, P, P, c_int, c_int, c_int, c_int, P]),
    "avc_vit_ln_bwd": (c_int, [P, P, P, c_float, P, P, P, c_int, c_int, P]),
    "avc_vit_attention_fwd_packed": (c_int, [P, P, c_int, c_int, c_int, c_int, P]),
    "avc_vit_attention_fwd": (c_int, [P, P, c_int, c_int, c_int, c_int, P]),
    "avc_vit_attention_bwd": (c_int, [P, P, P, c_int, c_int, c_int, c_int, P]),
    "avc_probe_mfma": (c_int, [P, P, P, P, P, P, P]),
    "avc_rasterize_faces": (c_int, [P, P, c_int, c_int, c_float, c_float, P, P, P]),
    "avc_rasterize_scratch_bytes": (c_long, [c_int, c_int]),
    "avc_rasterize_mesh": (c_int, [P, c_int, P, c_int, P, c_float, P, c_int, c_float, c_float, P, P, c_int, c_int, P, P]),
    "avc_rasterize_mesh_save": (c_int, [P, c_int, c_int, P, c_int, P, c_float, P, c_int, c_float, c_float, P, P, P, P, P]),
    "avc_rasterize_mesh_grad": (c_int, [P, P, c_int, c_int, P, c_int, P, P, c_int, c_float, P, P, P, P, P, P]),
    "avc_dense_params_fwd": (c_int, [c_int, P, P, P, P, P, P, P, P, P]),
    "avc_dense_params_bwd": (c_int, [c_int, P, P, P, P, P, P, P, P, P, P, P]),
    "avc_weight_grad_all": (c_int, [P, c_int, P, c_int, c_int, P, c_long, P, P, c_int, c_int, c_int, P]),
    "avc_weight_grad_reduce": (c_int, [P, P, c_int, c_int, c_int, c_int, c_int, P, c_int, P]),
    "avc_weight_grad_unpack": (c_int, [P, P, P, P, c_int, P, P]),
    "avc_shade_loss_blocks": (c_int, [c_int]),
    "avc_shade_loss_fwd": (c_int, [P, P, P, P, P, P, P, P, c_float, P, c_int, c_int, P, P, P, P, P]),
    "avc_colsum": (c_int, [P, c_long, c_int, c_int, P, P, P]),
    "avc_colsum_scratch_bytes": (c_long, []),
    "avc_inv_s": (c_int, [P, P, P, P]),
    "avc_pack_params": (c_int, [P, c_int, P, P, c_int, P, P, c_int, P, P, P, P]),
    "avc_coarse_z": (c_int, [P, P, P, c_int, c_int, P, P]),
    "avc_loss_tail_fwd": (c_int, [P, P, c_int, c_int, c_int, P, P, c_float, c_float, c_float, c_float, P, P, P, P]),
    "avc_loss_tail_bwd": (c_int, [P, P, P, c_int, c_int, c_int, P, P, c_float, c_float, c_float, c_float, P, P, P]),
    "avc_shade_loss_bwd": (c_int, [P, P, P, P, P, P, P, P, c_int, c_int, P, P, P, P, P, P, P, P]),
    "avc_resize_norm_fwd": (c_int, [P, c_int, c_int, c_int, P, P, P, P]),
    "avc_resize_norm_bwd": (c_int, [P, c_int, c_int, c_int, P, P, P, P]),
    "avc_gen_rays": (c_int, [P, P, P, c_int, c_int, c_float, c_float, c_float, c_int, c_int, c_int, P, P, P, P, P, P, P]),
    "avc_chess_background": (c_int, [P, c_int, c_int, c_int, P, P]),
    "avc_nearest_point": (c_int, [P, c_int, P, c_int, P, P]),
    "avc_mesh_components": (c_int, [P, c_int, c_int, P, P]),
    "avc_mesh_largest_island": (c_int, [P, c_int, c_int, P, P, P, P, P, P]),
    "avc_mesh_compact": (c_int, [P, P, P, c_int, c_int, P, P, P, P, P, P, P, P]),
    "avc_skin_apply": (c_int, [P, P, P, c_int, c_int, c_int, P, P]),
    "avc_rig_cell_keys": (c_int, [P, c_int, c_double, c_double, c_double, c_double, c_int, P, P]),
    "avc_rig_cluster_heads": (c_int, [P, c_int, P, P]),
    "avc_rig_cluster_average": (c_int, [P, c_int, P, P, c_int, P, c_int, P, P, P, P]),
    "avc_rig_tri_keys": (c_int, [P, c_int, c_int, P, c_int, P, P, P]),
    "avc_rig_tri_unique": (c_int, [P, P, c_int, P, P]),
    "avc_rig_tri_compact": (c_int, [P, c_int, P, P, c_int, P, P]),
    "avc_skin_sort_template": (c_int, [P, c_int, c_int, P, P, P, P]),
    "avc_skin_pack": (c_int, [P, P, P, c_int, P, c_int, c_int, P, P, P, P]),
    "avc_rot_to_quat": (c_int, [P, c_long, P, P]),
}
_OPTIONAL = {}
_RING_SIGS = {
    "avc_bwd_ring_ctl_bytes": (c_long, []),
    "avc_bwd_ring_payload_bytes": (c_long, [c_int, c_int, c_int]),
    "avc_bwd_ring_types": (c_int, [c_int]),
    "avc_render_points_bwd_ring": (c_int, [c_int, P, P, P, P, c_int, c_int, c_float, c_long, P, P, P, P, P, P, P, P, P, P, P,
                                           P, P, P, P, P, c_int, c_int, c_int, c_int, P]),
}


def lib_path():
    return _build.LIB


def load():
    global _lib
    if _lib is not None:
        return _lib
    path = lib_path()
    if not os.path.exists(path):
        raise RuntimeError("libavc.so is not built (run `python -c 'import __graft_entry__ as g; g.build()'`); "
                           "there is no CPU fallback for the HIP hot path")
    lib = ctypes.CDLL(path)
    lib.avc_last_error.restype = ctypes.c_char_p
    lib.avc_last_error.argtypes = []
    for name, (res, args) in list(_SIGS.items()) + list(_OPTIONAL.items()):
        fn = getattr(lib, name)
        fn.restype = res
        fn.argtypes = args
    for name, (res, args) in _RING_SIGS.items():
        if hasattr(lib, name):
            fn = getattr(lib, name)
            fn.restype = res
            fn.argtypes = args
    got = lib.avc_version()
    if got != ABI_VERSION:
        raise RuntimeError("%s implements revision %d of include/avc.h, this binding expects %d: rebuild the library "
                           "(python -m avatarclip_amd.build --force)" % (path, got, ABI_VERSION))
    _lib = lib
    return lib


def has_ring():
    return hasattr(load(), "avc_render_points_bwd_ring")


def register_optional(sigs):
    _OPTIONAL.update(sigs)


def ptr(t):
    if t is None:
        return None
    assert t.is_cuda and t.is_contiguous(), "HIP kernels need contiguous device tensors"
    return t.data_ptr()


def stream():
    return torch.cuda.current_stream().cuda_stream


def check(rc, what=""):
    if rc != 0:
        raise RuntimeError("libavc %s failed: %s" % (what, load().avc_last_error().decode()))
```

include/avc.h:

```cpp
#ifndef AVC_H
#define AVC_H
#ifdef __cplusplus
extern "C" {
#endif

#define AVC_NET_FULL 0
#define AVC_NET_SMALL 1

#define AVC_ABI_VERSION 3

const char* avc_last_error(void);
int avc_version(void);
int avc_num_offsets(void);

int avc_sdf_forward(int net, const float* pts, const float* rays_o, const float* rays_d, const float* z, int S,
                    int ldz, long npts, const void* wf16, const float* tab, const int* offs ,
                    float* sdf_out, const int* slot, int ld_out, void* stream);

int avc_upsample_step(const float* rays_o, const float* rays_d, const float* z_in, const float* sdf_in, int R,
                      int n, int m, float inv_s, float* z_out, float* sdf_out, float* z_new, int* slot_new,
                      void* stream);
int avc_upsample_step_lanes(const float* rays_o, const float* rays_d, const float* z_in, const float* sdf_in, int R,
                            int n, int m, float inv_s, float* z_out, float* sdf_out, float* z_new, int* slot_new,
                            int lanes_per_ray, void* stream);

int avc_render_points_fwd(int net, const float* pts, const float* rays_o, const float* rays_d, const float* z,
                          int S, int ldz, float sample_dist, long npts, const void* wf16, const float* tab,
                          const int* offs , float* sdf_out, float* normal_out, float* rgb_out, long max_waves,
                          void* scratch , void* stream);
long avc_fwd_scratch_bytes_per_wave(int net);

int avc_composite_fwd(const float* sdf, const float* normal, const float* rgb, const float* z, const float* rays_o,
                      const float* rays_d, int R, int S, const float* inv_s , float sample_dist,
                      float cos_anneal, const float* bg, int bg_mode, float* color, float* extra, float* weights,
                      float* cdf, float* mid_z, float* inside, float* eik, float* wstat, float* nsum, void* stream);

long avc_colsum_scratch_bytes(void);
int avc_colsum(const float* x, long R, int C, int mode, float* out, void* scratch, void* stream);
int avc_inv_s(const float* variance, const float* g, float* out, void* stream);

int avc_composite_bwd(const float* sdf, const float* normal, const float* rgb, const float* z, const float* rays_o,
                      const float* rays_d, int R, int S, const float* inv_s, float sample_dist, float cos_anneal,
                      const float* bg, int bg_mode, const float* d_color, const float* d_extra,
                      const float* d_weights, const float* d_normal_up, const float* d_wsum, const float* d_nsum,
                      const float* eik_scale, float* d_sdf, float* d_normal, float* d_rgb, float* d_inv_s, void* stream);

int avc_fwd_panel_tiles(int net);
int avc_grad_panel_tiles(int net);
int avc_mask_u16_per_block(int net);
int avc_render_points_fwd_train(int net, const float* pts, const float* rays_o, const float* rays_d, const float* z,
                                int S, int ldz, float sample_dist, long npts, const void* wf16, const float* tab,
                                const int* offs , float* sdf_out, float* normal_out, float* rgb_out,
                                long max_waves, void* fpanels, void* masks, void* stream);

int avc_bwd_colsum_floats(int net);
long avc_bwd_colsum_rows(long npts, long max_waves);
int avc_render_points_bwd(int net, const float* pts, const float* rays_o, const float* rays_d, const float* z,
                          int S, int ldz, float sample_dist, long npts, const void* wbf16, const float* tab,
                          const int* offs , const float* d_sdf, const float* d_normal, const float* d_rgb,
                          const float* rgb_fwd, const void* fpanels, void* gpanels, const void* masks, float* colsum,
                          long max_waves, void* stream);

int avc_weight_grad_all(const void* fpanels, int ftiles, const void* gpanels, int gtiles, int npairs,
                        const int* pairs , long nblk, float* partial, float* bias_partial, int nsplit,
                        int out_stride, int bias_stride, void* stream);

int avc_weight_grad_reduce(const float* partial, const float* bias_partial, int nsplit, int out_stride, int bias_stride, int gout_size,
                           int gbias_size, float* acc, int accumulate, void* stream);
int avc_weight_grad_unpack(const float* acc, const int* off, const int* src, const float* scale, int nparam, float* grad, void* stream);

int avc_shade_loss_blocks(int P);
int avc_shade_loss_fwd(const float* color, const float* extra, const float* wsum, const float* nsum, const float* true_rgb,
                       const float* mask, const int* ray_of_pixel, const float* bg, float bg_const, const float* light, int P,
                       int img0_is_extra, float* images, float* partial, float* sums, unsigned* ticket, void* stream);
int avc_shade_loss_bwd(const float* color, const float* extra, const float* wsum, const float* nsum, const float* true_rgb,
                       const float* mask, const int* ray_of_pixel, const float* light, int P, int img0_is_extra, const float* dimg0,
                       const float* dimg1, const float* gs, float* dcolor, float* dextra, float* dwsum, float* dnsum, void* stream);
int avc_pack_params(const float* flat, int nparam, const long* idx16, const float* scale16, int n16, const long* idx32,
                    const float* scale32, int n32, void* w_f16, void* w_bf16, float* tab, void* stream);
int avc_coarse_z(const float* near_, const float* far_, const float* jitter, int R, int n, float* z, void* stream);
int avc_loss_tail_fwd(const float* enc, const float* text, int B, int T, int D, const float* sums, const float* eikonal, float igr_weight,
                      float mask_weight, float clip_weight, float P, float* loss, float* out, float* saved, void* stream);
int avc_loss_tail_bwd(const float* g, const float* enc, const float* text, int B, int T, int D, const float* sums, const float* saved,
                      float igr_weight, float mask_weight, float clip_weight, float P, float* d_enc, float* dd, void* stream);
int avc_resize_norm_fwd(const float* images, int B, int H, int W, const float* mean, const float* stdv, float* out, void* stream);
int avc_resize_norm_bwd(const float* dout, int B, int H, int W, const float* mean, const float* stdv, float* dimages, void* stream);

int avc_gen_rays(const float* pose, const long* sel, const float* prior, int Hp, int Wp, float W, float H, float focal, int Wn, int Hn,
                 int R, float* rays_o, float* rays_d, float* near, float* far, float* true_rgb, float* mask, void* stream);
int avc_chess_background(float* out, int H, int W, int chess_length, const float* taps, void* stream);

int avc_dense_params_fwd(int n, const void* const* v, const void* const* g, const void* const* b, const int* rows,
                         const int* cols, const long* w_off, const long* b_off, float* flat, void* stream);
int avc_dense_params_bwd(int n, const void* const* v, const void* const* g, void* const* dv, void* const* dg, void* const* db,
                         const int* rows, const int* cols, const long* w_off, const long* b_off, const float* dflat,
                         void* stream);

int avc_mc_classify(const float* u, int nx, int ny, int nz, float iso, const int* ntri_table, int* vflag, int* ccount,
                    void* stream);
int avc_mc_emit(const float* u, int nx, int ny, int nz, float iso, const int* vflag, const int* vid, const int* ccount,
                const int* coff, const signed char* tri_table, const int* edge_table, float* verts, int* tris, void* stream);

int avc_vit_linear(const float* x, const void* w_packed, const float* bias, const float* residual, float* y,
                   float* y_pre, int M, int N, int K, int act, void* workspace ,
                   void* stream);
int avc_vit_linear_bwd_gelu(const float* dy, const float* pre, const void* wt_packed, float* dx, int M, int N, int K,
                            void* workspace, void* stream);
long avc_vit_workspace_bytes(int M, int K);
int avc_vit_ln_pack(const float* x, const float* gamma, const float* beta, float eps, int M, int K, void* xs_packed, void* stream);
int avc_vit_linear_packed(const void* xs_packed, const void* w_packed, const float* bias, const float* residual, float* y,
                          void* ys_packed, int M, int N, int K, int act, void* stream);
int avc_vit_attention_fwd_packed(const float* qkv, void* out_packed, int B, int T, int width, int heads, void* stream);
int avc_vit_pack(const float* x, const float* gelu_pre, void* xs_packed, int M, int K, void* stream);
int avc_vit_attention_bwd_packed(const float* qkv, const float* dout, void* dqkv_packed, int B, int T, int width, int heads, void* stream);
int avc_vit_linear_small(const void* xs_packed, const void* w_packed, const float* bias, const float* residual, const float* gelu_pre,
                         float* y, float* y_pre, void* ys_packed, int M, int N, int K, int act, void* stream);
int avc_vit_ln_bwd(const float* dy, const float* x, const float* gamma, float eps, const float* residual_grad, float* dx,
                   void* xs_packed, int M, int K, void* stream);
int avc_vit_attention_fwd(const float* qkv, float* out, int B, int T, int width, int heads, void* stream);
int avc_text_attention_fwd(const float* qkv, float* out, int B, int T, int width, int heads, int causal, void* stream);
int avc_vit_attention_bwd(const float* qkv, const float* dout, float* dqkv, int B, int T, int width, int heads,
                          void* stream);

int avc_probe_mfma(const void* a_f16, const void* b_f16, float* d, const void* a_bf16, const void* b_bf16, float* d_bf,
                   void* stream);

int avc_rasterize_mesh(const float* v_world, int V, const int* idx, int F, const float* cam, float width, const float* light, int S,
                       float near_, float far_, float* ndc, float* out, int flip_x, int channels, void* scratch, void* stream);
long avc_rasterize_scratch_bytes(int F, int image_size);
int avc_rasterize_faces(const float* faces, const float* light, int F, int image_size, float near_, float far_,
                        float* image, void* scratch , void* stream);

int avc_rasterize_mesh_save(const float* v_world, int N, int V, const int* idx, int F, const float* cam, float width, const float* light, int S,
                            float near_, float far_, float* ndc, float* image, int* fidx, void* scratch, void* stream);
int avc_rasterize_mesh_grad(const float* grad_image, const float* ndc, int N, int V, const int* idx, int F, const float* light, const int* fidx,
                            int S, float eps, const int* vf_ptr, const int* vf_ent, float* face_grad, float* grad_ndc, float* grad_light,
                            void* stream);

int avc_nearest_point(const float* q, int M, const float* ref, int K, int* idx, void* stream);
int avc_mesh_components(const int* tris, int F, int NV, int* label, void* stream);
int avc_mesh_largest_island(const int* tris, int F, int NV, const int* label, int* count, unsigned long long* best, int* vflag, int* tflag,
                            void* stream);
int avc_mesh_compact(const float* v, const unsigned* colors, const int* tris, int F, int NV, const int* vflag, const int* vid, const int* tflag,
                     const int* tid, float* v_out, unsigned* c_out, int* t_out, void* stream);
int avc_skin_apply(const float* xf, const int* idx, const float* p, int M, int K, int T, float* out, void* stream);

#define AVC_RIG_MAX_DIVISOR 1022
int avc_rig_cell_keys(const float* v, int N, double ox, double oy, double oz, double voxel_size, int voxel_divisor, long long* keyed,
                      void* stream);
int avc_rig_cluster_heads(const long long* sorted, int N, int* first_flag, void* stream);
int avc_rig_cluster_average(const long long* sorted, int N, const float* v, const unsigned char* colors, int csize, const int* first_rank,
                            int M, float* v_out, float* c_out, int* vmap, void* stream);
#define AVC_RIG_MAX_KEYED_VERTICES (1 << 21)
#define AVC_RIG_TRI_DROP 0x7FFFFFFFFFFFFFFFLL
int avc_rig_tri_keys(const int* tris, int F, int N, const int* vmap, int M, int* tri_out, long long* key, void* stream);
int avc_rig_tri_unique(const long long* sorted_key, const long long* order, int F, int* tflag, void* stream);
int avc_rig_tri_compact(const int* tri_in, int F, const int* tflag, const int* tid, int F_out, int* t_out, void* stream);
int avc_skin_sort_template(const float* weights, int K, int keep, unsigned char* tj, float* tw, int* count, void* stream);
int avc_skin_pack(const float* weights, const unsigned char* tj, const float* tw, int K, const int* nearest, int M, int sets,
                  unsigned char* joints, float* wout, float* blend_weights, void* stream);
int avc_rot_to_quat(const float* R, long n, float* q, void* stream);

#ifdef __cplusplus
}
#endif
#endif
```

Before: 2.282 million.

## Recompute delta2 tiles inside weight-grad kernel instead of storing them

The backward sweep kernel gets a variant that skips writing the delta2 gradient tiles to the global panels. The weight-gradient kernel's delta2×r1 pair instead rebuilds those tiles on the fly from the output-gradient tile, the relu masks and the head weights, using one MFMA per wave and a software-pipelined prefetch of the auxiliary data into LDS. The aim is to cut global write and read traffic for the delta2 panels. In exchange it adds extra MMA work, a larger LDS slot footprint and more complex pipelining in the weight-grad loop.

```diff
diff --git a/avatarclip_amd/csrc/avc_bwd_body.h b/avatarclip_amd/csrc/avc_bwd_body.h
--- a/avatarclip_amd/csrc/avc_bwd_body.h
+++ b/avatarclip_amd/csrc/avc_bwd_body.h
@@ -116,7 +116,7 @@
   template <class N> __device__ __forceinline__ void handoff(int, const b8 (&)[N::HK], long, int, int) const {}
 };
 
-template <class N, bool PIPE = false, class R>
+template <class N, bool PIPE = false, bool STORE_D2 = true, class R>
 __device__ __forceinline__ void bwd_sweeps(StageT<BWD_G>& sg, const BwdArgs& a, lds_tab_t Tl, long blk0, long nblk, int lane0,
                                            int wv, R& ring, cs_slot_t cs, BlkIn<N>* bip = nullptr, long blk0_next = 0) {
   typedef PanelLayout<N> L;
@@ -154,20 +154,20 @@
     for (int t = 0; t < N::HT; ++t) { m1[t] = bi.m1[t]; m2[t] = bi.m2[t]; }
     const float dn_in[3] = {bi.dn[0], bi.dn[1], bi.dn[2]};
     dsdf_in = bi.dsdf;
-#define AVC_RELU_BWD(OUT, MSK, PT)                                                                         \
+#define AVC_RELU_BWD(OUT, MSK, PT, STORE)                                                                  \
   AVC_EPI(const unsigned bits = MSK[t];                                                                      \
           _Pragma("unroll") for (int j = 0; j < 8; ++j) {                                                    \
             OUT[2 * t][j] = (__bf16)(((bits >> relu_mask_bit(j)) & 1u) ? acc[j] : 0.f);                      \
             OUT[2 * t + 1][j] = (__bf16)(((bits >> relu_mask_bit(8 + j)) & 1u) ? acc[8 + j] : 0.f); }        \
           pin2(OUT[2 * t], OUT[2 * t + 1]);                                                                  \
-          tile_store<false>(tiles, (PT) + t, OUT[2 * t], OUT[2 * t + 1]);)
+          if constexpr (STORE) tile_store<false>(tiles, (PT) + t, OUT[2 * t], OUT[2 * t + 1]);)
     b8 dl[N::HK];
     b8 d1[N::HK];
     if constexpr (N::NCMID == 1) {
-      layer_s1<b8, 1, N::HT>(sg, Wb, o.v[OFF_CHT], nxt<N, OFF_CM0T>(sg, Wb, o), dof, AVC_RELU_BWD(dl, m2, L::G_D2));
-      layer_s1<b8, N::HK, N::HT>(sg, Wb, o.v[OFF_CM0T], nxt<N, OFF_C0T>(sg, Wb, o), dl, AVC_RELU_BWD(d1, m1, L::G_D1));
+      layer_s1<b8, 1, N::HT>(sg, Wb, o.v[OFF_CHT], nxt<N, OFF_CM0T>(sg, Wb, o), dof, AVC_RELU_BWD(dl, m2, L::G_D2, STORE_D2));
+      layer_s1<b8, N::HK, N::HT>(sg, Wb, o.v[OFF_CM0T], nxt<N, OFF_C0T>(sg, Wb, o), dl, AVC_RELU_BWD(d1, m1, L::G_D1, true));
     } else {
-      layer_s1<b8, 1, N::HT>(sg, Wb, o.v[OFF_CHT], nxt<N, OFF_C0T>(sg, Wb, o), dof, AVC_RELU_BWD(d1, m1, L::G_D1));
+      layer_s1<b8, 1, N::HT>(sg, Wb, o.v[OFF_CHT], nxt<N, OFF_C0T>(sg, Wb, o), dof, AVC_RELU_BWD(d1, m1, L::G_D1, true));
     }
     float dn_acc[3] = {0.f, 0.f, 0.f};
     layer_s1<b8, N::HK, N::HT + 1>(sg, Wb, o.v[OFF_C0T], nxt<N, OFF_W0G>(sg, Wb, o), d1, AVC_EPI(
diff --git a/avatarclip_amd/csrc/avc_mlp_bwd.hip b/avatarclip_amd/csrc/avc_mlp_bwd.hip
--- a/avatarclip_amd/csrc/avc_mlp_bwd.hip
+++ b/avatarclip_amd/csrc/avc_mlp_bwd.hip
@@ -1,7 +1,7 @@
 #include "avc_bwd_body.h"
 #include "../../include/avc.h"
 
-template <class N>
+template <class N, bool STORE_D2>
 __global__ __launch_bounds__(64 * BWD_WPB) void mlp_bwd_kernel(BwdArgs a) {
   extern __shared__ __attribute__((aligned(16))) char lds[];
   typedef StageT<BWD_G> ST;
@@ -19,7 +19,7 @@
   BlkIn<N> bi;
   load_blk_in<N>(a, (long)blockIdx.x * BWD_WPB + wv, nblk, lane0, bi);
   for (long blk0 = (long)blockIdx.x * BWD_WPB; blk0 < nblk; blk0 += (long)gridDim.x * BWD_WPB)
-    bwd_sweeps<N, true>(sg, a, Tl, blk0, nblk, lane0, wv, ring, cs, &bi, blk0 + (long)gridDim.x * BWD_WPB);
+    bwd_sweeps<N, true, STORE_D2>(sg, a, Tl, blk0, nblk, lane0, wv, ring, cs, &bi, blk0 + (long)gridDim.x * BWD_WPB);
   cs_flush<N>(cs, a.colsum, (long)blockIdx.x * BWD_WPB + wv, lane0);
 }
 
@@ -33,11 +33,12 @@
   return grid * BWD_WPB;
 }
 
-extern "C" int avc_render_points_bwd(int net, const float* pts, const float* rays_o, const float* rays_d, const float* z,
+static int render_points_bwd(bool store_d2, const char* what, int net, const float* pts, const float* rays_o, const float* rays_d, const float* z,
                                      int S, int ldz, float sample_dist, long npts, const void* wbf16, const float* tab,
                                      const int* offs, const float* d_sdf, const float* d_normal, const float* d_rgb,
                                      const float* rgb_fwd, const void* fpanels, void* gpanels, const void* masks, float* colsum,
                                      long max_waves, void* stream) {
+  if (!store_d2 && net != AVC_NET_FULL) { avc_set_error("avc_render_points_bwd_nod2: the net has no delta2 tiles (no middle colour layer)"); return 1; }
   if (npts <= 0) return 0;
   if (!fpanels || !gpanels || !masks || !rgb_fwd || !colsum) { avc_set_error("avc_render_points_bwd: fpanels / gpanels / masks / rgb_fwd / colsum == NULL"); return 1; }
   if (!(net == AVC_NET_FULL ? offsets_match<NetFull>(offs) : offsets_match<NetSmall>(offs))) {
@@ -56,15 +57,34 @@
   if (offs[OFF_TAB_END] * 4 > AVC_TAB_LDS_BYTES) { avc_set_error("fp32 table does not fit its LDS window"); return 1; }
   static unsigned long long attr_seen = 0;
   if (avc_first_use_on_device(attr_seen)) {
-    (void)hipFuncSetAttribute((const void*)mlp_bwd_kernel<NetFull>, hipFuncAttributeMaxDynamicSharedMemorySize, lds_bytes);
-    (void)hipFuncSetAttribute((const void*)mlp_bwd_kernel<NetSmall>, hipFuncAttributeMaxDynamicSharedMemorySize, lds_bytes);
+    (void)hipFuncSetAttribute((const void*)mlp_bwd_kernel<NetFull, true>, hipFuncAttributeMaxDynamicSharedMemorySize, lds_bytes);
+    (void)hipFuncSetAttribute((const void*)mlp_bwd_kernel<NetFull, false>, hipFuncAttributeMaxDynamicSharedMemorySize, lds_bytes);
+    (void)hipFuncSetAttribute((const void*)mlp_bwd_kernel<NetSmall, true>, hipFuncAttributeMaxDynamicSharedMemorySize, lds_bytes);
   }
   const BwdArgs args{ps, npts, (const b8*)wbf16, tab, d_sdf, d_normal, d_rgb, rgb_fwd, (const char*)fpanels, (char*)gpanels,
                      (const unsigned short*)masks, colsum};
-  if (net == AVC_NET_FULL)
-    hipLaunchKernelGGL((mlp_bwd_kernel<NetFull>), dim3(grid), dim3(64 * BWD_WPB), lds_bytes, s, args);
+  if (net == AVC_NET_FULL && store_d2)
+    hipLaunchKernelGGL((mlp_bwd_kernel<NetFull, true>), dim3(grid), dim3(64 * BWD_WPB), lds_bytes, s, args);
+  else if (net == AVC_NET_FULL)
+    hipLaunchKernelGGL((mlp_bwd_kernel<NetFull, false>), dim3(grid), dim3(64 * BWD_WPB), lds_bytes, s, args);
   else if (net == AVC_NET_SMALL)
-    hipLaunchKernelGGL((mlp_bwd_kernel<NetSmall>), dim3(grid), dim3(64 * BWD_WPB), lds_bytes, s, args);
+    hipLaunchKernelGGL((mlp_bwd_kernel<NetSmall, true>), dim3(grid), dim3(64 * BWD_WPB), lds_bytes, s, args);
   else { avc_set_error("unknown net id"); return 1; }
-  return avc_check_launch("avc_render_points_bwd");
+  return avc_check_launch(what);
 }
+extern "C" int avc_render_points_bwd(int net, const float* pts, const float* rays_o, const float* rays_d, const float* z,
+                                     int S, int ldz, float sample_dist, long npts, const void* wbf16, const float* tab,
+                                     const int* offs, const float* d_sdf, const float* d_normal, const float* d_rgb,
+                                     const float* rgb_fwd, const void* fpanels, void* gpanels, const void* masks, float* colsum,
+                                     long max_waves, void* stream) {
+  return render_points_bwd(true, "avc_render_points_bwd", net, pts, rays_o, rays_d, z, S, ldz, sample_dist, npts, wbf16, tab, offs, d_sdf,
+                           d_normal, d_rgb, rgb_fwd, fpanels, gpanels, masks, colsum, max_waves, stream);
+}
+extern "C" int avc_render_points_bwd_nod2(int net, const float* pts, const float* rays_o, const float* rays_d, const float* z,
+                                          int S, int ldz, float sample_dist, long npts, const void* wbf16, const float* tab,
+                                          const int* offs, const float* d_sdf, const float* d_normal, const float* d_rgb,
+                                          const float* rgb_fwd, const void* fpanels, void* gpanels, const void* masks, float* colsum,
+                                          long max_waves, void* stream) {
+  return render_points_bwd(false, "avc_render_points_bwd_nod2", net, pts, rays_o, rays_d, z, S, ldz, sample_dist, npts, wbf16, tab, offs,
+                           d_sdf, d_normal, d_rgb, rgb_fwd, fpanels, gpanels, masks, colsum, max_waves, stream);
+}
diff --git a/avatarclip_amd/csrc/avc_wgrad.hip b/avatarclip_amd/csrc/avc_wgrad.hip
--- a/avatarclip_amd/csrc/avc_wgrad.hip
+++ b/avatarclip_amd/csrc/avc_wgrad.hip
@@ -2,11 +2,21 @@
 #include "../../include/avc.h"
 
 #include "avc_wgrad_body.h"
-
-template <int NI, int NK>
+#include "avc_mlp.h"
+
+struct WgRebuild {
+  const char* wht;
+  const char* aux_do;
+  const char* aux_mk;
+  long mask_stride;
+};
+constexpr int WG_AUX_TILE = 16;
+
+template <int NI, int NK, bool RB = false>
 __device__ __forceinline__ void weight_grad_body(char* lds, const WgRegions& rg, int pa, int ta_n, int pb,
                                                  int tb_n, int type_a, int type_b, long nblk, float* __restrict__ partial,
-                                                 float* __restrict__ bias_partial, int out_elems, int bias_elems, int WA) {
+                                                 float* __restrict__ bias_partial, int out_elems, int bias_elems, int WA,
+                                                 const WgRebuild& rb = WgRebuild{}) {
   const int lane = threadIdx.x & 63;
   const int wv = __builtin_amdgcn_readfirstlane((int)(threadIdx.x >> 6));
   const int WB = 8 / WA;
@@ -14,21 +24,61 @@
   const int split = blockIdx.x, nsplit = gridDim.x;
   const long b0 = nblk * split / nsplit, b1 = nblk * (split + 1) / nsplit;
   const int ntile = ta_n + tb_n;
-  const int nchunk = ntile * 2;
+  const int nchunk = RB ? tb_n * 2 + 2 : ntile * 2;
   const int my_chunks = (nchunk - wv + 7) >> 3;
   constexpr int slot_bytes = WG_BUF_BYTES, depth = WG_DEPTH;
   const int src_lo = ((lane >> 2) & 3) * 32 + 4 * (lane >> 4) + (lane & 3);
   const char* const base_a = (type_a ? rg.base[1] : rg.base[0]) + (long)pa * 2048;
   const char* const base_b = (type_b ? rg.base[1] : rg.base[0]) + (long)pb * 2048;
   const long stride_a = type_a ? rg.stride[1] : rg.stride[0], stride_b = type_b ? rg.stride[1] : rg.stride[0];
+  auto issue_aux = [&](int c, long blk, int slot) {
+    const char* g = (c ? rb.aux_mk + blk * rb.mask_stride : rb.aux_do + blk * stride_a) + lane * 16;
+    __builtin_amdgcn_global_load_lds((const __attribute__((address_space(1))) void*)g,
+                                     (__attribute__((address_space(3))) void*)(lds + slot * slot_bytes + WG_AUX_TILE * 2048 + c * 1024), 16, 0, WG_DMA_AUX);
+  };
   auto issue = [&](long blk, int slot) {
     for (int c = wv; c < nchunk; c += 8) {
-      const int tix = c >> 1;
-      const char* tb_ = tix < ta_n ? base_a + blk * stride_a + (long)tix * 2048 : base_b + blk * stride_b + (long)(tix - ta_n) * 2048;
-      const char* g = tb_ + (src_lo + (c & 1) * 16) * 16;
-      __builtin_amdgcn_global_load_lds((const __attribute__((address_space(1))) void*)g,
-                                       (__attribute__((address_space(3))) void*)(lds + slot * slot_bytes + c * 1024), 16, 0, WG_DMA_AUX);
-    }
+      if constexpr (RB) {
+        if (c < tb_n * 2) {
+          const char* g = base_b + blk * stride_b + (long)(c >> 1) * 2048 + (src_lo + (c & 1) * 16) * 16;
+          __builtin_amdgcn_global_load_lds((const __attribute__((address_space(1))) void*)g,
+                                           (__attribute__((address_space(3))) void*)(lds + slot * slot_bytes + (ta_n * 2 + c) * 1024), 16, 0, WG_DMA_AUX);
+        } else {
+          issue_aux(c - tb_n * 2, blk + 1 < b1 ? blk + 1 : blk, slot + 1 < depth ? slot + 1 : 0);
+        }
+      } else {
+        const int tix = c >> 1;
+        const char* tb_ = tix < ta_n ? base_a + blk * stride_a + (long)tix * 2048 : base_b + blk * stride_b + (long)(tix - ta_n) * 2048;
+        const char* g = tb_ + (src_lo + (c & 1) * 16) * 16;
+        __builtin_amdgcn_global_load_lds((const __attribute__((address_space(1))) void*)g,
+                                         (__attribute__((address_space(3))) void*)(lds + slot * slot_bytes + c * 1024), 16, 0, WG_DMA_AUX);
+      }
+    }
+  };
+  b8 wht = {};
+  if constexpr (RB) wht = *reinterpret_cast<const AVC_GLOBAL b8*>(as_global(rb.wht) + wv * 1024 + lane * 16);
+  struct Rebuilt { b8 dof; facc acc; unsigned bits; };
+  auto produce_read = [&](int slot, Rebuilt& r) {
+    lds_char* aux = (lds_char*)(lds + slot * slot_bytes) + WG_AUX_TILE * 2048;
+    r.dof = *reinterpret_cast<__attribute__((address_space(3))) b8*>(aux + lane * 16);
+    r.bits = *reinterpret_cast<__attribute__((address_space(3))) unsigned short*>(aux + 1024 + wv * 128 + lane * 2);
+  };
+  auto produce_mma = [&](Rebuilt& r) {
+#pragma unroll
+    for (int q = 0; q < 16; ++q) r.acc[q] = 0.f;
+    r.acc = MF<b8>::mma(wht, r.dof, r.acc);
+  };
+  auto produce_store = [&](int slot, const Rebuilt& r) {
+    b8 f0, f1;
+#pragma unroll
+    for (int j = 0; j < 8; ++j) {
+      f0[j] = (__bf16)(((r.bits >> relu_mask_bit(j)) & 1u) ? r.acc[j] : 0.f);
+      f1[j] = (__bf16)(((r.bits >> relu_mask_bit(8 + j)) & 1u) ? r.acc[8 + j] : 0.f);
+    }
+    const int p = lane & 31, hh = lane >> 5;
+    lds_char* dst = (lds_char*)(lds + slot * slot_bytes) + wv * 2048 + ((p >> 2) * 16 + hh * 4 + (p & 3)) * 16;
+    *reinterpret_cast<__attribute__((address_space(3))) b8*>(dst) = f0;
+    *reinterpret_cast<__attribute__((address_space(3))) b8*>(dst + 8 * 16) = f1;
   };
   const int lane_off = (((lane >> 5) * 2) * 16 + (((lane >> 4) & 1) * 2 + (lane & 1)) * 4 + ((lane & 15) >> 2)) * 16 + 8 * ((lane & 3) >> 1);
   facc acc[NI * NK];
@@ -39,8 +89,19 @@
   float bsum[NI];
 #pragma unroll
   for (int i = 0; i < NI; ++i) bsum[i] = 0.f;
+  if constexpr (RB) {
+    if (wv < 2 && b0 < b1) issue_aux(wv, b0, 0);
+  }
   for (int d = 0; d < depth - 1; ++d)
     if (b0 + d < b1) issue(b0 + d, d);
+  if constexpr (RB) {
+    long ahead = b1 - b0;
+    if (ahead > depth - 1) ahead = depth - 1;
+    wait_vmcnt((int)ahead * my_chunks);
+    __builtin_amdgcn_s_barrier();
+    __builtin_amdgcn_sched_barrier(0);
+    if (b0 < b1) { Rebuilt r; produce_read(0, r); produce_mma(r); produce_store(0, r); }
+  }
   int slot = 0;
   for (long blk = b0; blk < b1; ++blk) {
     long younger = b1 - 1 - blk;
@@ -49,7 +110,15 @@
     asm volatile("s_waitcnt lgkmcnt(0)" ::: "memory");
     __builtin_amdgcn_s_barrier();
     __builtin_amdgcn_sched_barrier(0);
+    const int nslot = slot + 1 < depth ? slot + 1 : 0;
+    Rebuilt nx;
+    if constexpr (RB) {
+      if (blk + 1 < b1) produce_read(nslot, nx);
+    }
     if (blk + depth - 1 < b1) { int ns = slot + depth - 1; if (ns >= depth) ns -= depth; issue(blk + depth - 1, ns); }
+    if constexpr (RB) {
+      if (blk + 1 < b1) produce_mma(nx);
+    }
     lds_char* buf = (lds_char*)(lds + slot * slot_bytes) + lane_off;
     b8 a[NI][2];
 #pragma unroll
@@ -92,6 +161,9 @@
           }
         }
       }
+    }
+    if constexpr (RB) {
+      if (blk + 1 < b1) produce_store(nslot, nx);
     }
     if (++slot == depth) slot = 0;
   }
@@ -261,11 +333,8 @@
 
 #define WG_MAX_PAIRS 24
 struct WgPairs { int v[WG_MAX_PAIRS][8]; };
-__global__ __launch_bounds__(512) void weight_grad_all_kernel(WgRegions rg, WgPairs pp, long nblk,
-                                                              float* __restrict__ partial, float* __restrict__ bias_partial,
-                                                              int out_elems, int bias_elems) {
-  extern __shared__ __attribute__((aligned(16))) char lds[];
-  const int* d = pp.v[blockIdx.y];
+__device__ __forceinline__ void weight_grad_pair(char* lds, const WgRegions& rg, const int* d, long nblk, float* __restrict__ partial,
+                                                 float* __restrict__ bias_partial, int out_elems, int bias_elems) {
   float* bp = d[5] >= 0 ? bias_partial + d[5] : nullptr;
 #define WG_ARGS lds, rg, d[0], d[1], d[2], d[3], d[6], d[7], nblk, partial + d[4], bp, out_elems, bias_elems
   if (d[1] > 1 && d[3] > 2 && d[3] <= 8) {
@@ -282,6 +351,24 @@
   }
 #undef WG_ARGS
 }
+__global__ __launch_bounds__(512) void weight_grad_all_kernel(WgRegions rg, WgPairs pp, long nblk,
+                                                              float* __restrict__ partial, float* __restrict__ bias_partial,
+                                                              int out_elems, int bias_elems) {
+  extern __shared__ __attribute__((aligned(16))) char lds[];
+  weight_grad_pair(lds, rg, pp.v[blockIdx.y], nblk, partial, bias_partial, out_elems, bias_elems);
+}
+__global__ __launch_bounds__(512) void weight_grad_all_kernel_rebuild(WgRegions rg, WgPairs pp, long nblk,
+                                                                      float* __restrict__ partial, float* __restrict__ bias_partial,
+                                                                      int out_elems, int bias_elems, WgRebuild rb) {
+  extern __shared__ __attribute__((aligned(16))) char lds[];
+  const int* d = pp.v[blockIdx.y];
+  if (d[6] == AVC_WG_TYPE_REBUILD) {
+    float* bp = d[5] >= 0 ? bias_partial + d[5] : nullptr;
+    weight_grad_body<4, 2, true>(lds, rg, d[0], d[1], d[2], d[3], 1, 0, nblk, partial + d[4], bp, out_elems, bias_elems, 2, rb);
+  } else {
+    weight_grad_pair(lds, rg, d, nblk, partial, bias_partial, out_elems, bias_elems);
+  }
+}
 
 extern "C" int avc_weight_grad_all(const void* fpanels, int ftiles, const void* gpanels, int gtiles, int npairs, const int* pairs,
                                    long nblk, float* partial, float* bias_partial, int nsplit, int out_stride, int bias_stride,
@@ -312,6 +399,65 @@
   return avc_check_launch("avc_weight_grad_all");
 }
 
+extern "C" int avc_weight_grad_all_rebuild(const void* fpanels, int ftiles, const void* gpanels, int gtiles, int npairs, const int* pairs,
+                                           long nblk, float* partial, float* bias_partial, int nsplit, int out_stride, int bias_stride,
+                                           const void* wbf16, const int* offs, const void* masks, void* stream) {
+  typedef PanelLayout<NetFull> PL;
+  static_assert(PL::HT == 8 && PL::NC == 1, "one wave per delta2 tile");
+  static_assert(2 * PL::HT < WG_AUX_TILE + 1 && WG_AUX_TILE < WG_TILES_MAX, "the aux tile lies behind the operand tiles, inside the slot");
+  if (nblk <= 0 || npairs <= 0) return 0;
+  if (!fpanels || !gpanels) { avc_set_error("avc_weight_grad_all_rebuild: fpanels / gpanels == NULL"); return 1; }
+  if (!wbf16 || !offs || !masks) { avc_set_error("avc_weight_grad_all_rebuild: wbf16 / offs / masks == NULL"); return 1; }
+  if (!offsets_match<NetFull>(offs)) {
+    avc_set_error("avc_weight_grad_all_rebuild: packed-blob offsets differ from the compiled-in table of the full nets");
+    return 1;
+  }
+  if (ftiles != PL::P_TILES || gtiles != PL::G_TILES) { avc_set_error("avc_weight_grad_all_rebuild: ftiles / gtiles are not the full nets' panel layout"); return 1; }
+  if (npairs > WG_MAX_PAIRS) { avc_set_error("avc_weight_grad_all_rebuild: too many pairs"); return 1; }
+  WgPairs pp;
+  int nrebuilt = 0;
+  for (int i = 0; i < npairs; ++i) {
+    for (int k = 0; k < 8; ++k) pp.v[i][k] = pairs[i * 8 + k];
+    const int* d = pp.v[i];
+    if (d[6] == AVC_WG_TYPE_REBUILD) {
+      if (d[0] != PL::G_D2 || d[1] != PL::HT || d[2] != PL::P_R1 || d[3] != PL::HT || d[7] != 0) {
+        avc_set_error("avc_weight_grad_all_rebuild: the rebuilt pair must be delta2 (G_D2, HT tiles) x r1 (P_R1, HT tiles, F region)");
+        return 1;
+      }
+      ++nrebuilt;
+      continue;
+    }
+    if ((d[6] != 0 && d[6] != 1) || (d[7] != 0 && d[7] != 1)) { avc_set_error("avc_weight_grad_all_rebuild: bad operand type"); return 1; }
+    if (d[6] == 1 && d[0] < PL::G_D2 + PL::HT && d[0] + d[1] > PL::G_D2) {
+      avc_set_error("avc_weight_grad_all_rebuild: a stored pair reads the delta2 tiles (they are not written; mark the pair as rebuilt)");
+      return 1;
+    }
+    const bool merged = d[1] == 9 && d[3] == 9;
+    if (!merged && (d[1] < 1 || d[1] > 8 || d[3] < 1 || d[3] > WG_TB_MAX)) {
+      avc_set_error("avc_weight_grad_all_rebuild: 1 <= ta <= 8, 1 <= tb <= 9 (or the 9 x 9 product)");
+      return 1;
+    }
+  }
+  if (nrebuilt != 1) { avc_set_error("avc_weight_grad_all_rebuild: the pair table needs exactly one rebuilt pair (type_a = AVC_WG_TYPE_REBUILD)"); return 1; }
+  if (nsplit < 1) nsplit = 1;
+  const int lds_bytes = WG_DEPTH * WG_BUF_BYTES;
+  static unsigned long long attr_seen = 0;
+  if (avc_first_use_on_device(attr_seen)) {
+    (void)hipFuncSetAttribute((const void*)weight_grad_all_kernel_rebuild, hipFuncAttributeMaxDynamicSharedMemorySize, lds_bytes);
+  }
+  WgRegions rg;
+  rg.base[0] = (const char*)fpanels; rg.stride[0] = (long)ftiles * 2048;
+  rg.base[1] = (const char*)gpanels; rg.stride[1] = (long)gtiles * 2048;
+  WgRebuild rb;
+  rb.wht = (const char*)wbf16 + (long)offs[OFF_CHT] * 2;
+  rb.aux_do = (const char*)gpanels + (long)PL::G_DO * 2048;
+  rb.aux_mk = (const char*)masks + (long)PL::HT * 64 * 2;
+  rb.mask_stride = (long)PL::MASK_U16 * 2;
+  hipLaunchKernelGGL(weight_grad_all_kernel_rebuild, dim3(nsplit, npairs), dim3(512), lds_bytes, (hipStream_t)stream, rg, pp, nblk, partial,
+                     bias_partial, out_stride, bias_stride, rb);
+  return avc_check_launch("avc_weight_grad_all_rebuild");
+}
+
 __global__ __launch_bounds__(256) void wgrad_reduce_kernel(const float* __restrict__ partial, const float* __restrict__ bpartial, int ns,
                                                            long stride, long bstride, int gout4, int gbias4, float* __restrict__ acc,
                                                            int accumulate) {
diff --git a/avatarclip_amd/engine.py b/avatarclip_amd/engine.py
--- a/avatarclip_amd/engine.py
+++ b/avatarclip_amd/engine.py
@@ -184,6 +184,8 @@
     PANEL_BYTES_BUDGET = int(os.environ.get("AVC_PANEL_GIB", "224")) << 30
     SLAB_BLOCKS = int(os.environ.get("AVC_SLAB_BLOCKS", str(512 * 1024)))
     MIN_SLAB_BLOCKS = 32 * 1024
+    STORE_D2 = False
+    WG_TYPE_REBUILD = 2
 
     def __init__(self, spec: PK.NetSpec, device):
         if device.type != "cuda":
@@ -209,6 +211,14 @@
         self._bpartials = None
         self._masks = None
         self._pairs_host = PK.region_local_pairs(self.dl.lay)
+        self._pairs_rebuild = None
+        if spec.NCMID == 1:
+            lay, ht = self.dl.lay, spec.H // 32
+            d2 = lay.panel["D2"] - lay.panel["FTILES"]
+            rows = [i for i, pr in enumerate(self._pairs_host) if pr[6] == 1 and pr[0] == d2]
+            assert len(rows) == 1 and tuple(self._pairs_host[rows[0]][[1, 2, 3, 7]]) == (ht, lay.panel["R1"], ht, 0), "delta2 x r1: HT x HT tiles"
+            self._pairs_rebuild = self._pairs_host.copy()
+            self._pairs_rebuild[rows[0], 6] = self.WG_TYPE_REBUILD
         self._sdf_bias0 = int(self.dl.lay.pbase["sdf.b%d" % (spec.NMID + 2)])
         self._packed_key = None
         self._packed = None
@@ -451,7 +461,8 @@
         scratch_out = None
         if rg is not None:
             rg["err"].zero_()
-        pairs_host = rg["rest"] if rg is not None else self._pairs_host
+        rebuild = rg is None and not self.STORE_D2 and self._pairs_rebuild is not None
+        pairs_host = rg["rest"] if rg is not None else (self._pairs_rebuild if rebuild else self._pairs_host)
         cs_rows = int(self.lib.avc_bwd_colsum_rows(min(R, rays_per_slab) * S, self.MAX_BWD_WAVES)) if rg is None else 8 * rg["grid"]
         if self._colsum is None or self._colsum.shape[0] < cs_rows:
             self._colsum = torch.zeros(cs_rows, lay.cs_size, device=self.device, dtype=torch.float32)
@@ -480,7 +491,10 @@
                 if rg is None:
                     rows = int(self.lib.avc_bwd_colsum_rows(npts, self.MAX_BWD_WAVES))
                     with Engine._Timed("avc_render_points_bwd", npts):
-                        L.check(self.lib.avc_render_points_bwd(*bwd_args, self.MAX_BWD_WAVES, st), "avc_render_points_bwd")
+                        if rebuild:
+                            L.check(self.lib.avc_render_points_bwd_nod2(*bwd_args, self.MAX_BWD_WAVES, st), "avc_render_points_bwd_nod2")
+                        else:
+                            L.check(self.lib.avc_render_points_bwd(*bwd_args, self.MAX_BWD_WAVES, st), "avc_render_points_bwd")
                 else:
                     rows = 8 * rg["grid"]
                     self._colsum[:rows].zero_()
@@ -501,10 +515,13 @@
                 cs_total = cs_slab if cs_total is None else cs_total + cs_slab
                 ns = max(1, min(self.WG_MAX_SPLITS, nblk // self.WG_BLOCKS_PER_SPLIT, nblk))
                 with Engine._Timed("avc_weight_grad(all pairs)", npts):
-                    L.check(self.lib.avc_weight_grad_all(fptr, self.fwd_tiles, L.ptr(gpanels), self.grad_tiles, len(pairs_host),
-                                                         pairs_host.ctypes.data, nblk, L.ptr(self._partials),
-                                                         L.ptr(self._bpartials), ns, self._partials.stride(0),
-                                                         self._bpartials.stride(0), st), "avc_weight_grad_all")
+                    wg_args = (fptr, self.fwd_tiles, L.ptr(gpanels), self.grad_tiles, len(pairs_host), pairs_host.ctypes.data, nblk,
+                               L.ptr(self._partials), L.ptr(self._bpartials), ns, self._partials.stride(0), self._bpartials.stride(0))
+                    if rebuild:
+                        L.check(self.lib.avc_weight_grad_all_rebuild(*wg_args, L.ptr(pk.w_bf16), self.dl.offsets, mptr, st),
+                                "avc_weight_grad_all_rebuild")
+                    else:
+                        L.check(self.lib.avc_weight_grad_all(*wg_args, st), "avc_weight_grad_all")
                     if fused_tail:
                         L.check(self.lib.avc_weight_grad_reduce(L.ptr(self._partials), L.ptr(self._bpartials), ns, self._partials.stride(0),
                                                                 self._bpartials.stride(0), lay.gout_size, lay.gbias_size, L.ptr(gacc),
diff --git a/avatarclip_amd/lib.py b/avatarclip_amd/lib.py
--- a/avatarclip_amd/lib.py
+++ b/avatarclip_amd/lib.py
@@ -27,6 +27,7 @@
     "avc_grad_panel_tiles": (c_int, [c_int]),
     "avc_mask_u16_per_block": (c_int, [c_int]),
     "avc_render_points_bwd": (c_int, [c_int, P, P, P, P, c_int, c_int, c_float, c_long, P, P, P, P, P, P, P, P, P, P, P, c_long, P]),
+    "avc_render_points_bwd_nod2": (c_int, [c_int, P, P, P, P, c_int, c_int, c_float, c_long, P, P, P, P, P, P, P, P, P, P, P, c_long, P]),
     "avc_bwd_colsum_floats": (c_int, [c_int]),
     "avc_bwd_colsum_rows": (c_long, [c_long, c_long]),
     "avc_mc_classify": (c_int, [P, c_int, c_int, c_int, c_float, P, P, P, P]),
@@ -53,6 +54,7 @@
     "avc_dense_params_fwd": (c_int, [c_int, P, P, P, P, P, P, P, P, P]),
     "avc_dense_params_bwd": (c_int, [c_int, P, P, P, P, P, P, P, P, P, P, P]),
     "avc_weight_grad_all": (c_int, [P, c_int, P, c_int, c_int, P, c_long, P, P, c_int, c_int, c_int, P]),
+    "avc_weight_grad_all_rebuild": (c_int, [P, c_int, P, c_int, c_int, P, c_long, P, P, c_int, c_int, c_int, P, P, P, P]),
     "avc_weight_grad_reduce": (c_int, [P, P, c_int, c_int, c_int, c_int, c_int, P, c_int, P]),
     "avc_weight_grad_unpack": (c_int, [P, P, P, P, c_int, P, P]),
     "avc_shade_loss_blocks": (c_int, [c_int]),
diff --git a/include/avc.h b/include/avc.h
--- a/include/avc.h
+++ b/include/avc.h
@@ -60,10 +60,20 @@
                           const int* offs , const float* d_sdf, const float* d_normal, const float* d_rgb,
                           const float* rgb_fwd, const void* fpanels, void* gpanels, const void* masks, float* colsum,
                           long max_waves, void* stream);
+int avc_render_points_bwd_nod2(int net, const float* pts, const float* rays_o, const float* rays_d, const float* z,
+                               int S, int ldz, float sample_dist, long npts, const void* wbf16, const float* tab,
+                               const int* offs , const float* d_sdf, const float* d_normal, const float* d_rgb,
+                               const float* rgb_fwd, const void* fpanels, void* gpanels, const void* masks, float* colsum,
+                               long max_waves, void* stream);
 
 int avc_weight_grad_all(const void* fpanels, int ftiles, const void* gpanels, int gtiles, int npairs,
                         const int* pairs , long nblk, float* partial, float* bias_partial, int nsplit,
                         int out_stride, int bias_stride, void* stream);
+#define AVC_WG_TYPE_REBUILD 2
+int avc_weight_grad_all_rebuild(const void* fpanels, int ftiles, const void* gpanels, int gtiles, int npairs,
+                                const int* pairs , long nblk, float* partial, float* bias_partial, int nsplit,
+                                int out_stride, int bias_stride, const void* wbf16, const int* offs ,
+                                const void* masks, void* stream);
 
 int avc_weight_grad_reduce(const float* partial, const float* bias_partial, int nsplit, int out_stride, int bias_stride, int gout_size,
                            int gbias_size, float* acc, int accumulate, void* stream);
```

New measurement: 2.281 million. About the same (-0.0%).
